# opentrack/neuralnet-tracker-traincode

Hardware: AMD Instinct MI355X
Metric: face-crops/sec fwd+bwd @ batch 512 (higher is better)
Workload: dtype f32; 1 GPU; NetworkWithPointHead(mobilenetv1, point head on, NLL off = training-script defaults): zero_grad + fwd + multi-task loss + bwd + fused clip/Adam step; per_gpu_batch=512, global_batch=512, input=129x129x1 f32, parallelism=dp1

## Files before the change

include/ttk.h:

```cpp
#ifndef TTK_H_
#define TTK_H_

#include <stddef.h>
#include <stdint.h>

#ifdef __cplusplus
extern "C" {
#endif

typedef void* ttk_stream_t;

#define TTK_ABI_VERSION 31

enum {
  TTK_BN_SCALE = 0,
  TTK_BN_BETA = 1,
  TTK_BN_MEAN = 2,
  TTK_BN_RSTD = 3,
  TTK_BN_GA = 4,
  TTK_BN_GB = 5,
  TTK_BN_GMEAN = 6,
  TTK_BN_AUX = 7,
  TTK_BN_ROWS = 8
};
enum { TTK_AUX_ACT_BOUND = 0, TTK_AUX_DY_BOUND = 1, TTK_AUX_GMAX = 2 };
#define TTK_STORE_ACT_BF16 1
#define TTK_STORE_GRAD_BF16 2
#define TTK_LAYOUT_ROWS 4
#define TTK_LAYOUT_CB64 8
#define TTK_MAX_PARTIAL_ROWS_ELEMENTWISE 1024
#define TTK_GEMM_BLOCK_M 128

int ttk_abi_version(void);
const char* ttk_last_error_string(void);
int ttk_clear_error(void);

int ttk_partial_rows_elementwise(int64_t work_items);
int ttk_partial_rows_dwconv(int B, int H, int W, int C, int stride, int backward);
int ttk_partial_rows_gemm(int64_t M);
int ttk_partial_rows_pwconv(int64_t M, int K, int Nout, int dgrad);
int ttk_pwconv_tile_rows(int64_t M, int K, int Nout, int dgrad);

int ttk_bn_fwd_finalize(float* part, const float* pivot, int part_rows, int C, int64_t count,
                        const float* gamma, const float* beta,
                        float* running_mean, float* running_var, int64_t* num_batches_tracked,
                        float momentum, float eps, float* bn, ttk_stream_t stream);
int ttk_bn_eval_prepare(const float* gamma, const float* beta, const float* running_mean,
                        const float* running_var, float eps, int C, float* bn, ttk_stream_t stream);
int ttk_bn_bwd_finalize(float* part, int part_rows, int C, int64_t count, const float* gamma,
                        float* bn, float* dgamma, float* dbeta, int accumulate, ttk_stream_t stream);

int ttk_bn_bwd_frozen(float* bn, int C, ttk_stream_t stream);
int ttk_bn_frozen_bound(float* part, const float* pivot, int part_rows, int C, int64_t count, float* bn, ttk_stream_t stream);

int ttk_stem_fwd(const float* x, const float* w, void* y, float* part, const float* pivot, int B, int H, int W,
                 int act_bf16, ttk_stream_t stream);
size_t ttk_stem_wgrad_partial_bytes(void);
int ttk_stem_bwd_weight(const void* g, const void* y, const float* bn, const float* x, float* dw,
                        int accumulate, float* partial, int B, int H, int W, int act_bf16,
                        ttk_stream_t stream);

int ttk_dwconv3x3_fwd(const float* yprev, const float* bn_prev, const float* skip_prev, float* a_out,
                      const float* w, float* y, float* part, const float* pivot, int B, int H, int W, int C,
                      int stride, int act_bf16, ttk_stream_t stream);
int ttk_dwconv3x3_bwd_data(const float* g_dw, const float* y_dw, const float* bn_dw, const float* w,
                           const float* skip_grad, const float* yprev, float* bn_prev,
                           const float* skip_prev, const float* a_in, float* g_prev, float* part,
                           float* dw, int dw_accumulate, float* dw_partial, int B, int H, int W, int C,
                           int stride, int act_bf16, ttk_stream_t stream);

int ttk_pwconv1x1_fwd(const float* ydw, const float* bn_dw, const float* w, float* y, float* part, const float* pivot,
                      int64_t M, int Cin, int Cout, void* wsplit, int act_bf16, ttk_stream_t stream);
int ttk_pwconv1x1_bwd_data(const float* g, const float* y, const float* bn_pw, const float* wt,
                           const float* ydw, const float* bn_dw, float* g_dw, float* part, int64_t M,
                           int Cin, int Cout, void* wsplit, int act_bf16, ttk_stream_t stream);
size_t ttk_pwconv_wgrad_partial_bytes(int64_t M, int Cin, int Cout);
size_t ttk_pwconv_wgrad_scratch_bytes(int64_t M, int Cin, int Cout);
int ttk_pwconv1x1_bwd_weight(const float* g, const float* y, const float* bn_pw, const float* ydw,
                             const float* bn_dw, float* dw, float* partial, int64_t M, int Cin, int Cout,
                             int act_bf16, ttk_stream_t stream);
int ttk_pwconv1x1_bwd_fused_rows(int64_t M, int Cin, int Cout);
size_t ttk_pwconv1x1_bwd_fused_partial_bytes(int64_t M, int Cin, int Cout);
int ttk_pwconv1x1_bwd_fused(const float* g, const float* y, const float* bn_pw, const float* w, const void* wsplit,
                            const float* ydw, const float* bn_dw, float* g_dw, float* dw, float* partial, float* part,
                            int64_t M, int Cin, int Cout, ttk_stream_t stream);
size_t ttk_pwconv_prepared_bytes(int Cin, int Cout);
int ttk_pwconv_prepare_weights(int n, const float* const* w, const int* cin, const int* cout,
                               void* const* prepared, ttk_stream_t stream);
int ttk_transpose(const float* in, float* out, int rows, int cols, ttk_stream_t stream);

int ttk_avgpool_fwd(const float* y, const float* bn, const float* skip, float* feat, int B, int HW,
                    int C, int act_bf16, ttk_stream_t stream);
int ttk_avgpool_bwd(const float* gfeat, const float* y, float* bn, const float* skip, float* g,
                    float* part, int B, int HW, int C, int act_bf16, ttk_stream_t stream);
int ttk_bn_act(const float* y, const float* bn, const float* skip, float* a, int64_t rows, int C,
               ttk_stream_t stream);

int ttk_anyc_partial_rows(int64_t pixels);
int ttk_anyc_stem_fwd(const float* x, const float* w, float* y, float* part, const float* pivot, int B, int H, int W, int Cout,
                      ttk_stream_t stream);
size_t ttk_anyc_stem_wgrad_scratch_bytes(int B, int H, int W, int Cout);
int ttk_anyc_stem_bwd_weight(const float* g, const float* y, const float* bn, const float* x, float* dw, int accumulate, float* scratch, int B,
                             int H, int W, int Cout, ttk_stream_t stream);
int ttk_anyc_dw_fwd(const float* yprev, const float* bn_prev, const float* skip_prev, float* a_out, const float* w, float* y, float* part,
                    const float* pivot, int B, int H, int W, int C, int stride, ttk_stream_t stream);
size_t ttk_anyc_dw_wgrad_scratch_bytes(int B, int H, int W, int C);
int ttk_anyc_dw_bwd_data(const float* g_dw, const float* y_dw, const float* bn_dw, const float* w, const float* skip_grad, const float* yprev,
                         float* bn_prev, const float* skip_prev, const float* a_in, float* g_prev, float* part, float* dw, int dw_accumulate,
                         float* dw_scratch, int B, int H, int W, int C, int stride, ttk_stream_t stream);
int ttk_anyc_pw_fwd(const float* ydw, const float* bn_dw, const float* w, float* y, float* part, const float* pivot, int64_t M, int Cin, int Cout,
                    ttk_stream_t stream);
int ttk_anyc_pw_bwd_data(const float* g, const float* y, const float* bn_pw, const float* w, const float* ydw, float* bn_dw, float* g_dw,
                         float* part, int64_t M, int Cin, int Cout, ttk_stream_t stream);
size_t ttk_anyc_pw_wgrad_scratch_bytes(int64_t M, int Cin, int Cout);
int ttk_anyc_pw_bwd_weight(const float* g, const float* y, const float* bn_pw, const float* ydw, const float* bn_dw, float* dw, int accumulate,
                           float* scratch, int64_t M, int Cin, int Cout, ttk_stream_t stream);
int ttk_anyc_avgpool_fwd(const float* y, const float* bn, const float* skip, float* feat, int B, int HW, int C, ttk_stream_t stream);
int ttk_anyc_avgpool_bwd(const float* gfeat, const float* y, float* bn, const float* skip, float* g, float* part, int B, int HW, int C,
                         ttk_stream_t stream);
int ttk_anyc_bn_act(const float* y, const float* bn, const float* skip, float* a, int64_t rows, int C, ttk_stream_t stream);

size_t ttk_bc_prepared_bytes(int Cin, int Cout);
int ttk_bc_prepare_weights(int n, const float* const* w, const int* cin, const int* cout, void* const* prepared, ttk_stream_t stream);
int ttk_bc_partial_rows_pw(int64_t M, int K, int Nout);
int ttk_bc_partial_rows_dw(int B, int H, int W, int C, int stride, int backward);
int ttk_bc_pw_fwd(const void* ydw, const float* bn_dw, const void* wprep, void* y, float* part, const float* pivot, int64_t M, int Cin,
                  int Cout, ttk_stream_t stream);
int ttk_bc_pw_bwd_data(const void* g, const void* y, const float* bn_pw, const void* wprep, const void* ydw, const float* bn_dw,
                       void* g_dw, float* part, int64_t M, int Cin, int Cout, ttk_stream_t stream);
size_t ttk_bc_pw_wgrad_scratch_bytes(int64_t M, int Cin, int Cout);
int ttk_bc_pw_bwd_weight(const void* g, const void* y, const float* bn_pw, const void* ydw, const float* bn_dw, float* dw,
                         float* scratch, int64_t M, int Cin, int Cout, ttk_stream_t stream);
int ttk_bc_pw_wgrad_slices(int64_t M, int Cin, int Cout);
int ttk_bc_pw_bwd_fused_rows(int64_t M, int Cin, int Cout);
size_t ttk_bc_pw_bwd_fused_scratch_bytes(int64_t M, int Cin, int Cout);
int ttk_bc_pw_bwd_fused(const void* g, const void* y, const float* bn_pw, const void* wprep, const void* ydw, const float* bn_dw,
                        void* g_dw, float* dw, float* scratch, float* part, int64_t M, int Cin, int Cout, ttk_stream_t stream);
int ttk_bc_partial_rows_pool(int B, int HW, int C);
int ttk_bc_avgpool_fwd(const void* y, const float* bn, const void* skip, float* feat, int B, int HW, int C, ttk_stream_t stream);
int ttk_bc_avgpool_bwd(const float* gfeat, const void* y, const float* bn, const void* skip, void* g, float* part, int B, int HW, int C,
                       ttk_stream_t stream);
int ttk_bc_dw_fwd(const void* yprev, const float* bn_prev, const void* skip_prev, void* a_out, const float* w, void* y, float* part,
                  const float* pivot, int B, int H, int W, int C, int stride, ttk_stream_t stream);
int ttk_bc_dw_bwd_data(const void* g_dw, const void* y_dw, const float* bn_dw, const float* w, const void* skip_grad,
                       const void* yprev, const float* bn_prev, const void* skip_prev, const void* a_in, void* g_prev, float* part,
                       float* dw, int dw_accumulate, float* dw_partial, int B, int H, int W, int C, int stride, ttk_stream_t stream);
int ttk_bc_bn_bwd_finalize_fold(float* part, int part_rows, int C, int64_t count, const float* gamma, float* bn, float* dgamma, float* dbeta,
                                int accumulate, const float* fold_partial, int fold_rows, int64_t fold_n, float* fold_out, int fold_accumulate,
                                ttk_stream_t stream);

int ttk_conv_weight_repack(const float* w, void* w_fwd, void* w_bwd, int Cout, int Cin, int KH, int KW,
                           ttk_stream_t stream);
int ttk_conv_prepare_weights(int n, const float* const* w, void* const* w_fwd, void* const* w_bwd, const int* cout,
                             const int* cin, const int* ksize, ttk_stream_t stream);
int ttk_conv_fwd(const float* a_in, const float* a_bound, const void* w_fwd, float* y, float* part, const float* pivot, int B, int H,
                 int W, int Cin, int Cout, int KH, int KW, int stride, int pad, ttk_stream_t stream);
int ttk_conv_bwd_data(const float* g, const float* y, const float* bn, const void* w_bwd, const float* mask_y,
                      float* mask_bn, float* g_in, float* part, int B, int H, int W, int Cin, int Cout,
                      int KH, int KW, int stride, int pad, ttk_stream_t stream);
size_t ttk_conv_wgrad_partial_bytes(int B, int H, int W, int Cin, int Cout, int KH, int KW, int stride, int pad);
int ttk_conv_bwd_weight(const float* g, const float* y, const float* bn, const float* a_in, const float* a_bound, float* dw,
                        float* partial, int B, int H, int W, int Cin, int Cout, int KH, int KW, int stride, int pad, ttk_stream_t stream);

int ttk_stem7_fwd(const float* x, const float* w, float* y, float* part, const float* pivot, int B, int H, int W, ttk_stream_t stream);
size_t ttk_stem7_wgrad_partial_bytes(int B, int H, int W);
int ttk_stem7_bwd_weight(const float* g, const float* y, const float* bn, const float* x, float* dw, float* partial, int B,
                         int H, int W, ttk_stream_t stream);
int ttk_maxpool3x3s2_fwd(const float* y, float* bn, float* a, unsigned char* idx, int B, int H, int W, int C,
                         ttk_stream_t stream);
int ttk_maxpool3x3s2_bwd(const float* ga, const float* gb, const unsigned char* idx, const float* y, const float* bn,
                         float* g, float* part, int B, int H, int W, int C, ttk_stream_t stream);
int ttk_bn_add_act(const float* y, float* bn, const float* res, const float* res_bn, float* a, const float* res_bound,
                   int measure, int64_t rows, int C, ttk_stream_t stream);
int ttk_bn_bwd_apply(const float* g, const float* y, const float* bn, void* dy, int64_t rows, int C, ttk_stream_t stream);
int ttk_blur3x3_fwd(const float* a, float* t, int B, int H, int W, int C, int stride, ttk_stream_t stream);
int ttk_blur3x3_bwd(const float* ga, const float* gb, float* g, int B, int H, int W, int C, int stride, ttk_stream_t stream);
int ttk_residual_bwd(const float* ga, const float* gb, const float* a, const float* y, float* bn, const float* yd,
                     float* bnd, float* gs, float* part, float* partd, int64_t rows, int C, ttk_stream_t stream);

int ttk_heads_num_rows(int enable_uncertainty, int enable_point_head, int enable_6drot);
int ttk_heads_fwd(const float* feat, const float* wcat, const float* bcat, const int* ids,
                  const float* P, const float* Pk, const float* keypts, const float* keyeig, int B, int F,
                  int NZ, int enable_uncertainty, int enable_point_head, int use_offset, int enable_6drot,
                  float* z, float* roi, float* coord, float* rot, float* qu, float* Lc, float* Lr, float* pts,
                  float* shp, ttk_stream_t stream);
int ttk_heads_bwd(const float* feat, const float* wcat, const float* z, const int* ids, const float* P,
                  const float* Pk, const float* keypts, const float* keyeig, int B, int F, int NZ,
                  int enable_uncertainty, int enable_point_head, int use_offset, int enable_6drot,
                  const float* g_roi, const float* g_coord, const float* g_rot, const float* g_qu,
                  const float* g_Lc, const float* g_Lr, const float* g_pts, const float* g_shp, float* dz,
                  float* dprow, float* dfeat, float* dwcat, float* dbcat, float* dP, float* dPk,
                  ttk_stream_t stream);
int ttk_diag_scale_fwd(const float* hidden, float* out, int n, ttk_stream_t stream);
int ttk_diag_scale_bwd(const float* hidden, const float* gout, float* ghidden, int n, ttk_stream_t stream);

int ttk_loss_rot_fwd(const float* q, const float* t, int n, float* v, ttk_stream_t stream);
int ttk_loss_rot_bwd(const float* q, const float* t, const float* gv, int n, float* gq, ttk_stream_t stream);
int ttk_loss_rot6d_fwd(const float* R, const float* t, int n, float* v, ttk_stream_t stream);
int ttk_loss_rot6d_bwd(const float* t, const float* gv, int n, float* gR, ttk_stream_t stream);
int ttk_loss_ortho6d_fwd(const float* z6, int n, float* v, ttk_stream_t stream);
int ttk_loss_ortho6d_bwd(const float* z6, const float* gv, int n, float* gz6, ttk_stream_t stream);
int ttk_mat_to_quat_fwd(const float* m, int n, float* q, ttk_stream_t stream);
int ttk_mat_to_quat_bwd(const float* m, const float* gq, int n, float* gm, ttk_stream_t stream);
int ttk_loss_quatreg_fwd(const float* q, int n, float* v, ttk_stream_t stream);
int ttk_loss_quatreg_bwd(const float* q, const float* gv, int n, float* gq, ttk_stream_t stream);
int ttk_loss_mse_rows_fwd(const float* p, const float* t, int n, int D, float* v, ttk_stream_t stream);
int ttk_loss_mse_rows_bwd(const float* p, const float* t, const float* gv, int n, int D, float* gp, ttk_stream_t stream);
int ttk_loss_mse_cols_fwd(const float* p, const float* t, int n, int Dt, int c0, int Dc, float* v, ttk_stream_t stream);
int ttk_loss_mse_cols_bwd(const float* p, const float* t, const float* gv, int n, int Dt, int c0, int Dc, float* gp, ttk_stream_t stream);
int ttk_multi_copy(int n, const float* const* src, float* const* dst, const int64_t* count, ttk_stream_t stream);
int ttk_weighted_sum_fwd(int n, const float* const* val, const float* const* sample_w, const float* w, const int* count,
                         float scale, float* out, ttk_stream_t stream);
int ttk_weighted_sum_bwd(int n, const float* gout, const float* const* sample_w, const float* w, const int* count,
                         float scale, float* const* gval, ttk_stream_t stream);
int ttk_loss_points_fwd(const float* p, const float* t, int n, int dim, float chin, float eye, float* v, ttk_stream_t stream);
int ttk_loss_points_bwd(const float* p, const float* t, const float* gv, int n, int dim, float chin, float eye, float* gp, ttk_stream_t stream);
int ttk_loss_nllrot_fwd(const float* q, const float* t, const float* L, int n, float* v, ttk_stream_t stream);
int ttk_loss_nllrot_bwd(const float* q, const float* t, const float* L, const float* gv, int n, float* gq, float* gL, ttk_stream_t stream);
int ttk_loss_nllcoord_fwd(const float* c, const float* t, const float* L, int n, float* v, ttk_stream_t stream);
int ttk_loss_nllcoord_bwd(const float* c, const float* t, const float* L, const float* gv, int n, float* gc, float* gL, ttk_stream_t stream);
int ttk_loss_normal_fwd(const float* mu, const float* sigma, const float* x, int n, int per, int points, int dim, float chin, float eye, float* v, ttk_stream_t stream);
int ttk_loss_normal_bwd(const float* mu, const float* sigma, const float* x, const float* gv, int n, int per, int points, int dim, float chin, float eye, float* gmu, float* gsigma, ttk_stream_t stream);
enum { TTK_ELEM_L2 = 0, TTK_ELEM_L1 = 1, TTK_ELEM_SMOOTH_L1 = 2 };
int ttk_loss_laplace_fwd(const float* mu, const float* b, const float* x, int n, int per, int points, int dim, float chin, float eye, float* v, ttk_stream_t stream);
int ttk_loss_laplace_bwd(const float* mu, const float* b, const float* x, const float* gv, int n, int per, int points, int dim, float chin, float eye, float* gmu, float* gb, ttk_stream_t stream);
int ttk_loss_elem_fwd(const float* p, const float* t, const float* colw, int n, int D, int kind, float beta, float* v, ttk_stream_t stream);
int ttk_loss_elem_bwd(const float* p, const float* t, const float* colw, const float* gv, int n, int D, int kind, float beta, float* gp, ttk_stream_t stream);
int ttk_loss_rot_geodesic_fwd(const float* q, const float* t, int n, float* v, ttk_stream_t stream);
int ttk_loss_rot_geodesic_bwd(const float* q, const float* t, const float* gv, int n, float* gq, ttk_stream_t stream);
int ttk_loss_gmm_fwd(const float* x, const double* ck, const double* mu, const double* sinv, int K, double fudge, int n, float* v, double* post, ttk_stream_t stream);
int ttk_loss_gmm_bwd(const float* x, const double* mu, const double* sinv, const double* post, int K, double fudge, const float* gv, int n, float* gx, ttk_stream_t stream);

#define TTK_LOSS_BATCH_MAX 32
enum {
  TTK_OP_ROT_FWD, TTK_OP_ROT_BWD, TTK_OP_ROT6D_FWD, TTK_OP_ROT6D_BWD, TTK_OP_ORTHO6D_FWD, TTK_OP_ORTHO6D_BWD,
  TTK_OP_QUATREG_FWD, TTK_OP_QUATREG_BWD, TTK_OP_MSE_ROWS_FWD, TTK_OP_MSE_ROWS_BWD, TTK_OP_MSE_COLS_FWD, TTK_OP_MSE_COLS_BWD,
  TTK_OP_POINTS_FWD, TTK_OP_POINTS_BWD, TTK_OP_NLLROT_FWD, TTK_OP_NLLROT_BWD, TTK_OP_NLLCOORD_FWD, TTK_OP_NLLCOORD_BWD,
  TTK_OP_NORMAL_FWD, TTK_OP_NORMAL_BWD, TTK_OP_GMM_FWD, TTK_OP_GMM_BWD, TTK_OP_COUNT
};
typedef struct ttk_loss_op {
  int kind;
  int items;
  const void* p[6];
  int i[4];
  float f[2];
  double d;
} ttk_loss_op;
int ttk_loss_batch(int nops, const ttk_loss_op* ops, ttk_stream_t stream);

int ttk_loss_batch_rows(int nops, const ttk_loss_op* ops, const unsigned* tag_sets, const int* tag_code, ttk_stream_t stream);
int ttk_row_weights(const float* wtable, const int* tag_code, const float* dataset_weight, int K, int n, float* rw, ttk_stream_t stream);

#define TTK_INTENSITY_EQUALIZE 0
#define TTK_INTENSITY_POSTERIZE_BITS 1
#define TTK_INTENSITY_GAMMA 2
#define TTK_INTENSITY_CONTRAST 3
#define TTK_INTENSITY_BRIGHTNESS 4
#define TTK_INTENSITY_BLUR 5
#define TTK_INTENSITY_NOISE_STD 6
#define TTK_INTENSITY_PARAMS 8
int ttk_intensity_augment(const float* x, float* y, const float* params, const float* noise, int B, int H, int W,
                          float out_shift, ttk_stream_t stream);

#define TTK_ADAM_MAX_GROUPS 128
#define TTK_ADAM_HYPER_LR 0
#define TTK_ADAM_HYPER_WD 128
#define TTK_ADAM_HYPER_FLOATS 256
int ttk_clip_adam(const int64_t* ptrs, const int32_t* numel, const int32_t* group,
                  const int32_t* chunk_tensor, const int32_t* chunk_offset, int nchunks, int chunk_size,
                  const float* lr4, const float* wd4, float beta1, float beta2, float eps, float max_norm,
                  float grad_scale, float* steps, float* partial, float* out_norm, const float* hyper_dev,
                  ttk_stream_t stream);

int ttk_view_roi(const float* face_roi, const float* scales, const float* translations,
                 float beyond_border_shift, int B, int* view_roi, ttk_stream_t stream);
int ttk_roi_transform(const int* view_roi, const float* angles, int B, int N, float* tr, ttk_stream_t stream);
int ttk_affine_warp(const void* src, int src_is_u8, int B, int Hs, int Ws, const float* tr, float* out,
                    int N, float mul, float add, ttk_stream_t stream);
int ttk_area_crop(const void* src, int src_is_u8, int B, int Hs, int Ws, const float* tr, float* out,
                  int N, float mul, float add, ttk_stream_t stream);
int ttk_affine_labels(const float* tr, int B, int N, float* coord, float* pose, float* roi,
                      const float* pts_in, float* pts_out, ttk_stream_t stream);

int ttk_stream_probe(const float* src, float* dst, float* sink, int64_t rows, int row_bytes, int seg_bytes, int nread, int nwrite,
                     int64_t stream_bytes, int unroll, int nontemporal, int blocks, ttk_stream_t stream);

#ifdef __cplusplus
}
#endif
#endif
```

neuralnet-tracker-traincode_amd/csrc/dwconv_tiled.hip:

```cpp
#include "ttk_common.h"
#include <type_traits>
#ifndef TTK_DW_FWD_U
#define TTK_DW_FWD_U 6
#endif
#ifndef TTK_DW_BWD_U
#define TTK_DW_BWD_U 4
#endif
#ifndef TTK_DW_FWD_U2
#define TTK_DW_FWD_U2 6
#endif

namespace ttk {

#ifndef TTK_DW_LDS_PIX
#define TTK_DW_LDS_PIX 368
#endif
constexpr int kLdsPixBudget32 = TTK_DW_LDS_PIX;
__host__ __device__ constexpr int lds_pix_budget(int SL) { return kLdsPixBudget32 * 32 / SL; }
__host__ __device__ constexpr int ilog2(int v) { return v <= 1 ? 0 : 1 + ilog2(v >> 1); }
#ifndef TTK_DW_WGS_PER_CU
#define TTK_DW_WGS_PER_CU 3
#endif
constexpr int kMaxDwBlocks = 256 * TTK_DW_WGS_PER_CU;
constexpr int kFwdUSkip = 4, kFwdUPlain = TTK_DW_FWD_U, kFwdUPlain2 = TTK_DW_FWD_U2;

struct DwTiling {
  int SL;
  int R, nbands, nslabs, grid, rows;
  int NI;
  int stage_rows;
  int NCT, TW;
  int carry;
};
#ifndef TTK_DW_CARRY
#define TTK_DW_CARRY 1
#endif
#ifndef TTK_DW_CARRY_BWD
#define TTK_DW_CARRY_BWD 1
#endif
constexpr int kCarryRegs = 5;

constexpr int kColTileMinW = 48;
constexpr int kColTile = 17;

__host__ __device__ inline int dw_band_rows(int Hgrid, int Wstage, int stride, bool backward, int SL = 32) {
  const int stage_rows = lds_pix_budget(SL) / (Wstage + 2);
  int R;
  if (!backward) R = (stage_rows - 3) / stride + 1;
  else R = (stride == 1) ? stage_rows - 2 : 2 * (stage_rows - 2);
  if (R < 1) R = 1;
  if (R > Hgrid) R = Hgrid;
  return R;
}

inline DwTiling dw_tiling_sl(int B, int H, int W, int C, int stride, bool backward, int SL) {
  const int Ho = (H - 1) / stride + 1, Wo = (W - 1) / stride + 1;
  DwTiling t;
  t.SL = SL;
  t.NCT = 1;
  t.TW = Wo;
  static const int col_tile = [] { const char* e = exp_env("TTK_DW_COLTILE"); return e ? atoi(e) : kColTile; }();
  static const int carry_bwd = [] { const char* e = exp_env("TTK_DW_CARRY_BWD"); return e ? atoi(e) : TTK_DW_CARRY_BWD; }();
  t.carry = backward ? (carry_bwd && stride == 1 && (Wo + 2) <= 80)
                     : (TTK_DW_CARRY && (3 - stride) * (W + 2) * (SL / 4) <= kCarryRegs * kBlock);
  if (!t.carry && stride == 1 && W >= kColTileMinW && col_tile < W) {
    t.NCT = (W + col_tile - 1) / col_tile;
    t.TW = (W + t.NCT - 1) / t.NCT;
  }
  const int Wtile = t.NCT > 1 ? t.TW : (backward ? Wo : W);
  t.R = backward ? dw_band_rows(H, Wtile, stride, true, SL) : dw_band_rows(Ho, Wtile, stride, false, SL);
  t.nbands = ((backward ? H : Ho) + t.R - 1) / t.R;
  t.nslabs = C / SL;
  t.stage_rows = backward ? (stride == 1 ? t.R + 2 : t.R / 2 + 2) : (t.R - 1) * stride + 3;
  t.NI = 1;
  if (t.nbands == 1) t.carry = 0;
  if (t.nbands == 1 && t.NCT == 1) {
    const int per_image = t.stage_rows * ((backward ? Wo : W) + 2);
    t.NI = lds_pix_budget(SL) / per_image;
    if (t.NI > B) t.NI = B;
    if (t.NI < 1) t.NI = 1;
  }
  int64_t tiles_per_slab = (int64_t)((B + t.NI - 1) / t.NI) * t.nbands * t.NCT;
  int64_t rows = kMaxDwBlocks / t.nslabs;
  if (rows < 1) rows = 1;
  if (rows > tiles_per_slab) rows = tiles_per_slab;
  t.rows = (int)rows;
  t.grid = t.rows * t.nslabs;
  return t;
}

inline DwTiling dw_tiling(int B, int H, int W, int C, int stride, bool backward) {
  return dw_tiling_sl(B, H, W, C, stride, backward, kCB);
}

struct TileDiv {
  float inv;
  unsigned d;
  __device__ __forceinline__ explicit TileDiv(unsigned d_) : inv(1.0f / (float)d_), d(d_) {}
  __device__ __forceinline__ unsigned div(unsigned n) const { return (unsigned)(((float)n + 0.5f) * inv); }
};

struct SlabWeights {
  float v[36];
  __device__ __forceinline__ void load(const float* w, int c) {
    const float4* p = reinterpret_cast<const float4*>(w + 9 * c);
#pragma unroll
    for (int i = 0; i < 9; ++i) {
      const float4 q = p[i];
      v[4 * i] = q.x; v[4 * i + 1] = q.y; v[4 * i + 2] = q.z; v[4 * i + 3] = q.w;
    }
  }
  __device__ __forceinline__ float4 tap(int t) const { return make_float4(v[t], v[9 + t], v[18 + t], v[27 + t]); }
};

template <int SL>
__device__ __forceinline__ float4 slab_wave_fold(float4 v) {
#pragma unroll
  for (int off = SL / 4; off < kWave; off <<= 1) {
    v.x += __shfl_xor(v.x, off); v.y += __shfl_xor(v.y, off);
    v.z += __shfl_xor(v.z, off); v.w += __shfl_xor(v.w, off);
  }
  return v;
}

struct D4 {
  double x, y, z, w;
  __device__ __forceinline__ void add(float4 v) { x += v.x; y += v.y; z += v.z; w += v.w; }
  __device__ __forceinline__ void addmul(float4 a, float4 b) {
    x += (double)a.x * b.x; y += (double)a.y * b.y; z += (double)a.z * b.z; w += (double)a.w * b.w;
  }
};
__device__ __forceinline__ double shfl_xor_d(double v, int off) {
  int lo = __double2loint(v), hi = __double2hiint(v);
  lo = __shfl_xor(lo, off);
  hi = __shfl_xor(hi, off);
  return __hiloint2double(hi, lo);
}
template <int SL>
__device__ __forceinline__ D4 slab_wave_fold_d(D4 v) {
#pragma unroll
  for (int off = SL / 4; off < kWave; off <<= 1) {
    v.x += shfl_xor_d(v.x, off); v.y += shfl_xor_d(v.y, off);
    v.z += shfl_xor_d(v.z, off); v.w += shfl_xor_d(v.w, off);
  }
  return v;
}

template <int SL>
__device__ __forceinline__ void slab_partials(D4 s1, D4 s2, int q, int C, int c_slab, float* part_row, float* red_f) {
  double* red = reinterpret_cast<double*>(red_f);
  s1 = slab_wave_fold_d<SL>(s1);
  s2 = slab_wave_fold_d<SL>(s2);
  const int lane = threadIdx.x & 63, wv = threadIdx.x >> 6;
  __syncthreads();
  if (lane < SL / 4) {
    double* d = red + (wv * 2 + 0) * SL + 4 * q;
    d[0] = s1.x; d[1] = s1.y; d[2] = s1.z; d[3] = s1.w;
    d = red + (wv * 2 + 1) * SL + 4 * q;
    d[0] = s2.x; d[1] = s2.y; d[2] = s2.z; d[3] = s2.w;
  }
  __syncthreads();
  if (threadIdx.x < 2 * SL) {
    const int which = threadIdx.x / SL, c = threadIdx.x % SL;
    double a = 0.0;
    for (int w = 0; w < kBlock / kWave; ++w) a += red[(w * 2 + which) * SL + c];
    part_row[(size_t)which * C + c_slab + c] = (float)a;
  }
}

template <int S, bool SKIP, int SL, bool CARRY>
__global__ void __launch_bounds__(kBlock) __attribute__((amdgpu_waves_per_eu(TTK_DW_WGS_PER_CU, TTK_DW_WGS_PER_CU)))
dw_fwd_tiled_k(const float* __restrict__ yprev, const float* __restrict__ bn_prev,
                                                          const float* __restrict__ skip_prev, float* __restrict__ a_out,
                                                          const float* __restrict__ w, float* __restrict__ y,
                                                          float* __restrict__ part, const float* __restrict__ pivot, int B, int H, int W, int C,
                                                          int Ho, int Wo, int R, int nbands, int nslabs, int NI_, int NCT_, int TW) {
  extern __shared__ __attribute__((aligned(16))) float lds[];
  constexpr int kSlab = SL, kSlabQuads = SL / 4, kPixSlots = kBlock / kSlabQuads, kQs = ilog2(kSlabQuads), kPs = ilog2(SL);
  const int tid = threadIdx.x, q = tid & (kSlabQuads - 1), slot = tid >> kQs;
  const int slab = blockIdx.x % nslabs, c0 = slab * kSlab + 4 * q;
  static_assert(SL == kCB, "a slab is one channel block of the activation layout");
  constexpr int cshift = 5;
  SlabWeights wr;
  wr.load(w, c0);
  const BnApply4 bn = BnApply4::load(bn_prev, C, c0);
  const float4 pv = pivot ? ld4(pivot + c0) : f4(0.f);
  D4 s1{0.0, 0.0, 0.0, 0.0}, s2{0.0, 0.0, 0.0, 0.0};
  const int NI = CARRY ? 1 : NI_, NCT = CARRY ? 1 : NCT_;
  constexpr bool carry = CARRY;
  const unsigned tiles = (unsigned)((B + NI - 1) / NI) * nbands * NCT;
  const unsigned wgs = gridDim.x / nslabs, wg = blockIdx.x / nslabs;
  const unsigned t_begin = carry ? (unsigned)((uint64_t)tiles * wg / wgs) : wg, t_end = carry ? (unsigned)((uint64_t)tiles * (wg + 1) / wgs) : tiles;
  const unsigned t_step = carry ? 1u : wgs;
  int prev_img = -1, prev_band = -2, prev_nrows = 0;
  constexpr int OV = 3 - S;
  for (unsigned t = t_begin; t < t_end; t += t_step) {
    const unsigned tb = t / (unsigned)NCT, ti = tb / (unsigned)nbands;
    const int ct = (int)(t - tb * NCT), band = (int)(tb - ti * nbands), n0 = (int)ti * NI;
    const int nimg = min(NI, B - n0);
    const int cx0 = ct * TW, tw = NCT > 1 ? min(TW, Wo - cx0) : Wo;
    const int Wp = NCT > 1 ? tw + 2 : W + 2;
    const int o0 = band * R, o1 = min(o0 + R, Ho);
    const int i0 = o0 * S - 1;
    const int nrows = (o1 - 1 - o0) * S + 3;
    const unsigned PI = (unsigned)(nrows * Wp);
    const TileDiv dPI(PI), dWp((unsigned)Wp), dtw((unsigned)tw);
    const size_t tin = ((size_t)slab * B * H * W + (size_t)n0 * H * W) * kCB, tout = ((size_t)slab * B * Ho * Wo + (size_t)n0 * Ho * Wo) * kCB;
    const float* ytile = yprev + tin;
    const float* sktile = SKIP ? skip_prev + tin : nullptr;
    float* aotile = a_out ? a_out + tin : nullptr;
    float* youttile = y + tout;
    const int ov = (carry && (int)ti == prev_img && band == prev_band + 1) ? OV : 0;
    const int own_hi = (carry && t + 1 < t_end && band + 1 < nbands) ? i0 + nrows : o1;
    float4 cr[kCarryRegs];
    const int ncopy = ov * Wp * kSlabQuads;
    if (ov) {
      const float* src = lds + (size_t)(prev_nrows - OV) * Wp * kSlab;
#pragma unroll
      for (int u = 0; u < kCarryRegs; ++u)
        if (tid + u * kBlock < ncopy) cr[u] = ld4(src + (size_t)(tid + u * kBlock) * 4);
    }
    prev_img = (int)ti; prev_band = band; prev_nrows = nrows;
    __syncthreads();
    if (ov) {
#pragma unroll
      for (int u = 0; u < kCarryRegs; ++u)
        if (tid + u * kBlock < ncopy) st4(lds + (size_t)(tid + u * kBlock) * 4, cr[u]);
    }
    const int nstage = nimg * ((int)PI - ov * Wp) * kSlabQuads;
    const unsigned ovpix = (unsigned)(ov * Wp);
    constexpr int kFwdU = SKIP ? kFwdUSkip : (S == 2 ? kFwdUPlain2 : (CARRY ? kFwdUPlain - 1 : kFwdUPlain));
    for (int e = tid; e < nstage; e += kFwdU * kBlock) {
      float4 yv[kFwdU], sk[SKIP ? kFwdU : 1];
      unsigned off[kFwdU];
      bool in[kFwdU];
      int pxs[kFwdU], rows[kFwdU];
#pragma unroll
      for (int u = 0; u < kFwdU; ++u) {
        const int ee = e + u * kBlock;
        const unsigned pxa = ((unsigned)ee >> kQs) + ovpix;
        const unsigned img = NI > 1 ? dPI.div(pxa) : 0u, px = NI > 1 ? pxa - __umul24(img, PI) : pxa;
        const unsigned prow = dWp.div(px);
        const int col = (int)(px - __umul24(prow, (unsigned)Wp)) - 1 + cx0, row = i0 + (int)prow;
        pxs[u] = (int)pxa;
        rows[u] = (row >= o0 && row < own_hi && col >= cx0 && col < cx0 + tw) ? 1 : 0;
        in[u] = ee < nstage && row >= 0 && row < H && col >= 0 && col < W;
        off[u] = in[u] ? ((__umul24(__umul24(img, (unsigned)H) + (unsigned)row, (unsigned)W) + (unsigned)col) << cshift) + 4 * q : 0u;
        yv[u] = in[u] ? ld4nt(ytile + off[u]) : f4(0.f);
        if constexpr (SKIP) sk[u] = in[u] ? ld4nt(sktile + off[u]) : f4(0.f);
      }
#pragma unroll
      for (int u = 0; u < kFwdU; ++u) {
        const int ee = e + u * kBlock;
        if (ee >= nstage) break;
        float4 a = f4(0.f);
        if (in[u]) {
          if constexpr (SKIP) a = bn.act(yv[u], sk[u]);
          else a = bn.act(yv[u]);
          if (S == 1 && a_out && rows[u]) st4(aotile + off[u], a);
        }
        st4(lds + (size_t)pxs[u] * kSlab + 4 * q, a);
      }
    }
    __syncthreads();
    const unsigned npix1 = (unsigned)((o1 - o0) * tw);
    const int npix = nimg * (int)npix1;
    const TileDiv dnp(npix1);
    for (int p = slot; p < npix; p += kPixSlots) {
      const unsigned img = NI > 1 ? dnp.div((unsigned)p) : 0u, pp = NI > 1 ? (unsigned)p - __umul24(img, npix1) : (unsigned)p;
      const unsigned prow = dtw.div(pp);
      const int ho = o0 + (int)prow, wl = (int)(pp - __umul24(prow, (unsigned)tw)), wo = cx0 + wl;
      const float* base = lds + ((__umul24(img, PI) + __umul24(prow * S, (unsigned)Wp) + (unsigned)(wl * S)) << kPs) + 4 * q;
      float4 acc = f4(0.f);
#pragma unroll
      for (int kh = 0; kh < 3; ++kh)
#pragma unroll
        for (int kw = 0; kw < 3; ++kw) acc = fma4(ld4(base + ((size_t)kh * Wp + kw) * kSlab), wr.tap(kh * 3 + kw), acc);
      st4(youttile + ((__umul24(__umul24(img, (unsigned)Ho) + (unsigned)ho, (unsigned)Wo) + (unsigned)wo) << cshift) + 4 * q, acc);
      acc = sub4(acc, pv);
      s1.add(acc);
      s2.addmul(acc, acc);
    }
  }
  if (part) {
    const int stage = NI * ((R - 1) * S + 3) * (NCT > 1 ? TW + 2 : W + 2) * kSlab;
    slab_partials<SL>(s1, s2, q, C, slab * kSlab, part + (size_t)(blockIdx.x / nslabs) * 2 * C, lds + stage);
  }
}

#ifndef TTK_DW_BWD_LEAN_PIX
#define TTK_DW_BWD_LEAN_PIX 4
#endif
#ifndef TTK_DW_BWD_LEAN_PIX2
#define TTK_DW_BWD_LEAN_PIX2 4
#endif
template <int S, int SL, bool LEAN, bool CARRY>
__global__ void __launch_bounds__(kBlock) __attribute__((amdgpu_waves_per_eu(TTK_DW_WGS_PER_CU, TTK_DW_WGS_PER_CU)))
dw_bwd_tiled_k(const float* __restrict__ g_dw, const float* __restrict__ y_dw,
                                                          const float* __restrict__ bn_dw, const float* __restrict__ w,
                                                          const float* __restrict__ skip_grad,
                                                          const float* __restrict__ yprev, float* __restrict__ bn_prev,
                                                          const float* __restrict__ skip_prev, const float* __restrict__ a_in,
                                                          float* __restrict__ g_prev, float* __restrict__ part,
                                                          float* __restrict__ dwgrad, float* __restrict__ dw_partial, int B, int H, int W, int C, int Ho, int Wo,
                                                          int R, int nbands, int nslabs, int stage_floats, int NI_, int NCT_, int TW, int ring) {
  extern __shared__ __attribute__((aligned(16))) float lds[];
  const int NI = CARRY ? 1 : NI_, NCT = CARRY ? 1 : NCT_;
  constexpr int kSlab = SL, kSlabQuads = SL / 4, kPixSlots = kBlock / kSlabQuads, kQs = ilog2(kSlabQuads), kPs = ilog2(SL);
  const int tid = threadIdx.x, q = tid & (kSlabQuads - 1), slot = tid >> kQs;
  const int slab = blockIdx.x % nslabs, c0 = slab * kSlab + 4 * q;
  float* wt = lds + stage_floats + 4 * 9 * kSlab;
  if (slot == 0) {
#pragma unroll
    for (int t = 0; t < 9; ++t)
      st4(wt + t * kSlab + 4 * q, make_float4(w[(size_t)(c0 + 0) * 9 + t], w[(size_t)(c0 + 1) * 9 + t], w[(size_t)(c0 + 2) * 9 + t], w[(size_t)(c0 + 3) * 9 + t]));
  }
  static_assert(SL == kCB, "a slab is one channel block of the activation layout");
  constexpr int cshift = 5;
  const BnApply4 bnp = BnApply4::load(bn_prev, C, c0);
  const BnGrad4 bg = BnGrad4::load(bn_dw, C, c0);
  D4 s1{0.0, 0.0, 0.0, 0.0}, s2{0.0, 0.0, 0.0, 0.0};
  float gmx = 0.f;
  float4 wacc[9];
#pragma unroll
  for (int t = 0; t < 9; ++t) wacc[t] = f4(0.f);
  const unsigned tiles = (unsigned)((B + NI - 1) / NI) * nbands * NCT;
  const unsigned wgs = gridDim.x / nslabs, wg = blockIdx.x / nslabs;
  const unsigned t_begin = CARRY ? (unsigned)((uint64_t)tiles * wg / wgs) : wg, t_end = CARRY ? (unsigned)((uint64_t)tiles * (wg + 1) / wgs) : tiles;
  const unsigned t_step = CARRY ? 1u : wgs;
  int prev_img = -1, prev_band = -2, prev_hi = -1;
  for (unsigned t = t_begin; t < t_end; t += t_step) {
    const unsigned tb = t / (unsigned)NCT, ti = tb / (unsigned)nbands;
    const int ct = (int)(t - tb * NCT), band = (int)(tb - ti * nbands), n0 = (int)ti * NI;
    const int nimg = min(NI, B - n0);
    const int cx0 = ct * TW, tw = NCT > 1 ? min(TW, W - cx0) : W;
    const int Wp = NCT > 1 ? tw + 2 : Wo + 2;
    const int r0 = band * R, r1 = min(r0 + R, H);
    const int ho_lo = max(0, (r0 - 1 + S - 1) / S * (r0 > 0 ? 1 : 0));
    const int ho_hi = min(Ho - 1, r1 / S);
    const int nrows = ho_hi - ho_lo + 1;
    const unsigned PI = (unsigned)(nrows * Wp);
    const TileDiv dPI(PI), dWp((unsigned)Wp), dtw((unsigned)tw);
    const size_t tdy = ((size_t)slab * B * Ho * Wo + (size_t)n0 * Ho * Wo) * kCB, tin = ((size_t)slab * B * H * W + (size_t)n0 * H * W) * kCB;
    const float* gtile = g_dw + tdy;
    const float* ydtile = y_dw + tdy;
    const float* yptile = yprev + tin;
    const float* aitile = a_in ? a_in + tin : nullptr;
    const float* sktile = skip_prev ? skip_prev + tin : nullptr;
    const float* sgtile = skip_grad ? skip_grad + tin : nullptr;
    float* gptile = g_prev + tin;
    const int ov = (CARRY && (int)ti == prev_img && band == prev_band + 1 && prev_hi >= ho_lo) ? prev_hi - ho_lo + 1 : 0;
    const int rbase = CARRY ? ho_lo % ring : 0;
    prev_img = (int)ti; prev_band = band; prev_hi = ho_hi;
    __syncthreads();
    const unsigned ovpix = (unsigned)(ov * Wp);
    const int nstage = nimg * ((int)PI - (int)ovpix) * kSlabQuads;
    constexpr int kBwdU = TTK_DW_BWD_U;
    for (int e = tid; e < nstage; e += kBwdU * kBlock) {
      float4 gv[kBwdU], yv[kBwdU];
      bool in[kBwdU];
      unsigned pxs[kBwdU];
#pragma unroll
      for (int u = 0; u < kBwdU; ++u) {
        const int ee = e + u * kBlock;
        const unsigned pxa = ((unsigned)ee >> kQs) + ovpix;
        const unsigned img = NI > 1 ? dPI.div(pxa) : 0u, px = NI > 1 ? pxa - __umul24(img, PI) : pxa;
        const unsigned prow = dWp.div(px);
        const int col = (int)(px - __umul24(prow, (unsigned)Wp)) - 1 + cx0, row = ho_lo + (int)prow;
        if constexpr (CARRY) {
          unsigned rr = (unsigned)rbase + prow;
          rr -= rr >= (unsigned)ring ? (unsigned)ring : 0u;
          pxs[u] = __umul24(rr, (unsigned)Wp) + (px - __umul24(prow, (unsigned)Wp));
        } else {
          pxs[u] = pxa;
        }
        in[u] = ee < nstage && col >= 0 && col < Wo;
        const unsigned off = in[u] ? ((__umul24(__umul24(img, (unsigned)Ho) + (unsigned)row, (unsigned)Wo) + (unsigned)col) << cshift) + 4 * q : 0u;
        gv[u] = in[u] ? ld4nt(gtile + off) : f4(0.f);
        yv[u] = in[u] ? ld4nt(ydtile + off) : f4(0.f);
      }
#pragma unroll
      for (int u = 0; u < kBwdU; ++u) {
        const int ee = e + u * kBlock;
        if (ee >= nstage) break;
        st4(lds + (size_t)pxs[u] * kSlab + 4 * q, in[u] ? bg.dy(gv[u], yv[u]) : f4(0.f));
      }
    }
    __syncthreads();
    const unsigned npix1 = (unsigned)((r1 - r0) * tw);
    const int npix = nimg * (int)npix1;
    const TileDiv dnp(npix1);
    constexpr int NP = LEAN ? (S == 2 ? TTK_DW_BWD_LEAN_PIX2 : TTK_DW_BWD_LEAN_PIX) : 2;
    for (int p = slot; p < npix; p += NP * kPixSlots) {
      bool has[NP];
      unsigned imgs[NP], offs[NP];
      int his[NP], wis[NP];
      float4 yps[NP], raws[NP], sgs[NP];
#pragma unroll
      for (int j = 0; j < NP; ++j) {
        const int pj = p + j * kPixSlots;
        has[j] = pj < npix;
        const unsigned pq = has[j] ? (unsigned)pj : (unsigned)p;
        imgs[j] = NI > 1 ? dnp.div(pq) : 0u;
        const unsigned pp = NI > 1 ? pq - __umul24(imgs[j], npix1) : pq;
        const unsigned pr = dtw.div(pp);
        his[j] = r0 + (int)pr;
        wis[j] = cx0 + (int)(pp - __umul24(pr, (unsigned)tw));
        offs[j] = ((__umul24(__umul24(imgs[j], (unsigned)H) + (unsigned)his[j], (unsigned)W) + (unsigned)wis[j]) << cshift) + 4 * q;
      }
#pragma unroll
      for (int j = 0; j < NP; ++j) yps[j] = ld4nt(yptile + offs[j]);
#pragma unroll
      for (int j = 0; j < NP; ++j) {
        raws[j] = f4(0.f);
        sgs[j] = f4(0.f);
        if (!LEAN) {
          if (a_in) raws[j] = ld4nt(aitile + offs[j]);
          else if (skip_prev) raws[j] = ld4nt(sktile + offs[j]);
          if (skip_grad) sgs[j] = ld4nt(sgtile + offs[j]);
        }
      }
#pragma unroll
      for (int j = 0; j < NP; ++j) {
        if (j > 0 && !has[j]) break;
        const int hi = his[j], wi = wis[j];
        const float* dyimg = lds + (__umul24(imgs[j], PI) << kPs);
        const float4 yp = yps[j], raw = raws[j], sg = sgs[j];
        float4 a;
        if (!LEAN && a_in) a = raw;
        else a = (!LEAN && skip_prev) ? bnp.act(yp, raw) : bnp.act(yp);
        float4 G = f4(0.f);
#pragma unroll
        for (int kh = 0; kh < 3; ++kh) {
          const int th = hi + 1 - kh;
          if (th < 0 || (S == 2 && (th & 1))) continue;
          const int ho = th / S;
          if (ho > Ho - 1) continue;
#pragma unroll
          for (int kw = 0; kw < 3; ++kw) {
            const int tw = wi + 1 - kw;
            if (S == 2 && (tw & 1)) continue;
            const int wo = (S == 1) ? tw : (tw >> 1);
            int lr = ho - ho_lo;
            if constexpr (CARRY) { lr += rbase; lr -= lr >= ring ? ring : 0; }
            const float4 dy = ld4(dyimg + ((__mul24(lr, Wp) + wo - cx0 + 1) << kPs) + 4 * q);
            G = fma4(dy, ld4(wt + (kh * 3 + kw) * kSlab + 4 * q), G);
            wacc[kh * 3 + kw] = fma4(dy, a, wacc[kh * 3 + kw]);
          }
        }
        if (!LEAN && skip_grad) G = add4(G, sg);
        const float4 gp = mask4(G, a);
        st4(gptile + offs[j], gp);
        gmx = fmaxf(fmaxf(gmx, fmaxf(fabsf(gp.x), fabsf(gp.y))), fmaxf(fabsf(gp.z), fabsf(gp.w)));
        s1.add(gp);
        s2.addmul(gp, sub4(yp, bnp.mean));
      }
    }
  }
  float* red = lds + stage_floats;
#pragma unroll
  for (int off = 32; off >= 1; off >>= 1) gmx = fmaxf(gmx, __shfl_xor(gmx, off));
  if ((tid & 63) == 0) {
    unsigned* slot = reinterpret_cast<unsigned*>(bn_prev + (size_t)TTK_BN_AUX * C + TTK_AUX_GMAX);
    if (__float_as_uint(gmx) > __hip_atomic_load(slot, __ATOMIC_RELAXED, __HIP_MEMORY_SCOPE_AGENT)) atomicMax(slot, __float_as_uint(gmx));
  }
  if (part) slab_partials<SL>(s1, s2, q, C, slab * kSlab, part + (size_t)(blockIdx.x / nslabs) * 2 * C, red);
  if (dwgrad) {
    __syncthreads();
    const int lane = tid & 63, wv = tid >> 6;
#pragma unroll
    for (int t = 0; t < 9; ++t) {
      const float4 v = slab_wave_fold<SL>(wacc[t]);
      if (lane < kSlabQuads) st4(red + ((size_t)wv * 9 + t) * kSlab + 4 * q, v);
    }
    __syncthreads();
    for (int i = tid; i < 9 * kSlab; i += kBlock) {
      const int t = i / kSlab, c = i % kSlab;
      float a = 0.f;
      for (int wq = 0; wq < kBlock / kWave; ++wq) a += red[((size_t)wq * 9 + t) * kSlab + c];
      if (dw_partial) dw_partial[((size_t)(blockIdx.x / nslabs) * C + slab * kSlab + c) * 9 + t] = a;
      else atomicAdd(dwgrad + (size_t)(slab * kSlab + c) * 9 + t, a);
    }
  }
}

__global__ void zero_fill_k(float* p, int64_t n) {
  const int64_t i = (int64_t)blockIdx.x * blockDim.x + threadIdx.x;
  if (i < n) p[i] = 0.f;
}

template <typename F>
static void with_flag(bool b, F&& f) {
  if (b) f(std::true_type{});
  else f(std::false_type{});
}

static bool dw_shape_ok2(int B, int H, int W, int C, int stride) {
  return B > 0 && H > 0 && W > 0 && W <= 256 && C >= 32 && C <= 1024 && (C & (C - 1)) == 0 && (stride == 1 || stride == 2);
}

}

using namespace ttk;

extern "C" {

int ttk_partial_rows_dwconv(int B, int H, int W, int C, int stride, int backward) {
  if (!dw_shape_ok2(B, H, W, C, stride)) return -1;
  return dw_tiling(B, H, W, C, stride, backward != 0).rows;
}

int ttk_dwconv3x3_fwd(const float* yprev, const float* bn_prev, const float* skip_prev, float* a_out, const float* w, float* y,
                      float* part, const float* pivot, int B, int H, int W, int C, int stride, int act_bf16, ttk_stream_t stream) {
  TTK_REQUIRE(yprev && bn_prev && w && y, "dwconv3x3_fwd: null pointer");
  TTK_REQUIRE(dw_shape_ok2(B, H, W, C, stride), "dwconv3x3_fwd: unsupported shape B=%d H=%d W=%d C=%d stride=%d (C: power of two in 32..1024, W <= 256)", B, H, W, C, stride);
  TTK_REQUIRE(!(a_out && stride != 1), "dwconv3x3_fwd: a_out requires stride 1");
  TTK_REQUIRE_FP32_STORAGE(act_bf16, "dwconv3x3_fwd");
  const int Ho = (H - 1) / stride + 1, Wo = (W - 1) / stride + 1;
  const DwTiling t = dw_tiling(B, H, W, C, stride, false);
  TTK_REQUIRE((int64_t)((B + t.NI - 1) / t.NI) * t.nbands * t.NCT < ((int64_t)1 << 31), "dwconv3x3_fwd: too many tiles for 32-bit indexing");
  const size_t stage = (size_t)t.NI * t.stage_rows * ((t.NCT > 1 ? t.TW : W) + 2) * t.SL;
  const size_t sm = (stage + 16 * t.SL) * sizeof(float);
  with_flag(stride == 2, [&](auto s2) {
    with_flag(skip_prev != nullptr, [&](auto skip) {
      with_flag(t.carry != 0, [&](auto carry) {
        hipLaunchKernelGGL((dw_fwd_tiled_k<decltype(s2)::value ? 2 : 1, decltype(skip)::value, kCB, decltype(carry)::value>), dim3(t.grid), dim3(kBlock), sm,
                           (hipStream_t)stream, yprev, bn_prev, skip_prev, a_out, w, y, part, pivot, B, H, W, C, Ho, Wo, t.R, t.nbands, t.nslabs, t.NI,
                           t.NCT, t.TW);
      });
    });
  });
  TTK_LAUNCH_CHECK("dwconv3x3_fwd");
}

int ttk_dwconv3x3_bwd_data(const float* g_dw, const float* y_dw, const float* bn_dw, const float* w, const float* skip_grad,
                           const float* yprev, float* bn_prev, const float* skip_prev, const float* a_in, float* g_prev,
                           float* part, float* dw, int dw_accumulate, float* dw_partial, int B, int H, int W, int C, int stride,
                           int act_bf16, ttk_stream_t stream) {
  TTK_REQUIRE(g_dw && y_dw && bn_dw && w && yprev && bn_prev && g_prev, "dwconv3x3_bwd_data: null pointer");
  TTK_REQUIRE(dw_shape_ok2(B, H, W, C, stride), "dwconv3x3_bwd_data: unsupported shape");
  TTK_REQUIRE(!(skip_grad && stride != 1), "dwconv3x3_bwd_data: residual gradient requires stride 1");
  TTK_REQUIRE_FP32_STORAGE(act_bf16, "dwconv3x3_bwd_data");
  const int Ho = (H - 1) / stride + 1, Wo = (W - 1) / stride + 1;
  const DwTiling t = dw_tiling(B, H, W, C, stride, true);
  TTK_REQUIRE((int64_t)((B + t.NI - 1) / t.NI) * t.nbands * t.NCT < ((int64_t)1 << 31), "dwconv3x3_bwd_data: too many tiles for 32-bit indexing");
  const size_t stage = (size_t)t.NI * t.stage_rows * ((t.NCT > 1 ? t.TW : Wo) + 2) * t.SL;
  const size_t sm = (stage + 4 * 9 * t.SL + 9 * t.SL) * sizeof(float);
  hipStream_t st = (hipStream_t)stream;
  if (!dw) dw_partial = nullptr;
  TTK_REQUIRE(dw_accumulate != 2 || dw_partial, "dwconv3x3_bwd_data: dw_accumulate = 2 (rows folded by the caller) needs dw and dw_partial");
  if (dw && !dw_accumulate && !dw_partial) hipLaunchKernelGGL(zero_fill_k, dim3((9 * C + 255) / 256), dim3(256), 0, st, dw, (int64_t)9 * C);
  with_flag(stride == 2, [&](auto s2) {
    with_flag(!a_in && !skip_prev && !skip_grad, [&](auto lean) {
      with_flag(t.carry != 0, [&](auto carry) {
        hipLaunchKernelGGL((dw_bwd_tiled_k<decltype(s2)::value ? 2 : 1, kCB, decltype(lean)::value, decltype(carry)::value>), dim3(t.grid), dim3(kBlock), sm, st,
                           g_dw, y_dw, bn_dw, w, skip_grad, yprev, bn_prev, skip_prev, a_in, g_prev, part, dw, dw_partial, B, H, W, C, Ho, Wo, t.R,
                           t.nbands, t.nslabs, (int)stage, t.NI, t.NCT, t.TW, t.stage_rows);
      });
    });
  });
  if (dw_partial && dw_accumulate != 2) launch_fold_partials(dw_partial, t.rows, (int64_t)9 * C, dw, dw_accumulate, st);
  TTK_LAUNCH_CHECK("dwconv3x3_bwd_data");
}

}
```

neuralnet-tracker-traincode_amd/csrc/pool.hip:

```cpp
#include "ttk_common.h"

namespace ttk {

__device__ __forceinline__ size_t pool_off(int layout, int64_t m, int c, int64_t M, int C) {
  if (layout == 1) return (size_t)m * C + c;
  if (layout == 2) return ((size_t)(c >> 6) * (size_t)M + (size_t)m) * 64 + (c & 63);
  return act_off(m, c, M);
}

__global__ void __launch_bounds__(kBlock) avgpool_fwd_k(const float* __restrict__ y, const float* __restrict__ bnp,
                                                         const float* __restrict__ skip,
                                                         float* __restrict__ feat, int B, int HW, int C, int rows_layout) {
  const int quads = C >> 2;
  const int64_t items = (int64_t)B * quads;
  const float inv = 1.0f / (float)HW;
  for (int64_t idx = (int64_t)blockIdx.x * kBlock + threadIdx.x; idx < items; idx += (int64_t)gridDim.x * kBlock) {
    const int c4 = (int)(idx % quads);
    const int n = (int)(idx / quads);
    const BnApply4 bn = BnApply4::load(bnp, C, 4 * c4);
    float4 s = f4(0.f);
    for (int p = 0; p < HW; ++p) {
      const int64_t m = (int64_t)n * HW + p;
      const size_t off = pool_off(rows_layout, m, 4 * c4, (int64_t)B * HW, C);
      s = add4(s, skip ? bn.act(ld4(y + off), ld4(skip + off)) : bn.act(ld4(y + off)));
    }
    st4(feat + (size_t)n * C + 4 * c4, make_float4(s.x * inv, s.y * inv, s.z * inv, s.w * inv));
  }
}

__global__ void __launch_bounds__(kBlock) avgpool_bwd_k(const float* __restrict__ gfeat, const float* __restrict__ y,
                                                         float* __restrict__ bnp, const float* __restrict__ skip, float* __restrict__ g,
                                                         float* __restrict__ part, int B, int HW, int C, int qshift, int rows_layout) {
  extern __shared__ __attribute__((aligned(16))) float smem[];
  const int quads = C >> 2;
  const int c4 = threadIdx.x & (quads - 1);
  const BnApply4 bn = BnApply4::load(bnp, C, 4 * c4);
  const float inv = 1.0f / (float)HW;
  const int64_t items = ((int64_t)B * HW) << qshift;
  float4 s1 = f4(0.f), s2 = f4(0.f);
  float gmx = 0.f;
  for (int64_t idx = (int64_t)blockIdx.x * kBlock + threadIdx.x; idx < items; idx += (int64_t)gridDim.x * kBlock) {
    const int n = (int)((unsigned)(idx >> qshift) / (unsigned)HW);
    const size_t off = pool_off(rows_layout, idx >> qshift, 4 * c4, (int64_t)B * HW, C);
    const float4 yv = ld4(y + off);
    const float4 a = skip ? bn.act(yv, ld4(skip + off)) : bn.act(yv);
    float4 gv = ld4(gfeat + (size_t)n * C + 4 * c4);
    gv = mask4(make_float4(gv.x * inv, gv.y * inv, gv.z * inv, gv.w * inv), a);
    st4(g + off, gv);
    gmx = fmaxf(fmaxf(gmx, fmaxf(fabsf(gv.x), fabsf(gv.y))), fmaxf(fabsf(gv.z), fabsf(gv.w)));
    s1 = add4(s1, gv);
    s2 = fma4(gv, sub4(yv, bn.mean), s2);
  }
#pragma unroll
  for (int off = 32; off >= 1; off >>= 1) gmx = fmaxf(gmx, __shfl_xor(gmx, off));
  if ((threadIdx.x & 63) == 0) {
    unsigned* slot = reinterpret_cast<unsigned*>(bnp + (size_t)TTK_BN_AUX * C + TTK_AUX_GMAX);
    if (__float_as_uint(gmx) > __hip_atomic_load(slot, __ATOMIC_RELAXED, __HIP_MEMORY_SCOPE_AGENT)) atomicMax(slot, __float_as_uint(gmx));
  }
  if (part) block_channel_partials<1024>(s1, s2, c4, C, part + (size_t)blockIdx.x * 2 * C, smem);
}

}

using namespace ttk;

static int pool_layout(int flags) { return (flags & TTK_LAYOUT_ROWS) ? 1 : ((flags & TTK_LAYOUT_CB64) ? 2 : 0); }

static int log2i_(int v) {
  int r = 0;
  while ((1 << r) < v) ++r;
  return r;
}

extern "C" {

int ttk_avgpool_fwd(const float* y, const float* bn, const float* skip, float* feat, int B, int HW,
                    int C, int act_bf16, ttk_stream_t stream) {
  TTK_REQUIRE(y && bn && feat, "avgpool_fwd: null pointer");
  TTK_REQUIRE(B > 0 && HW > 0 && C >= 32 && C <= 1024 && (C & (C - 1)) == 0, "avgpool_fwd: unsupported shape B=%d HW=%d C=%d", B, HW, C);
  TTK_REQUIRE_FP32_STORAGE(act_bf16, "avgpool_fwd");
  const int64_t items = (int64_t)B * (C / 4);
  hipLaunchKernelGGL(avgpool_fwd_k, dim3(elementwise_grid(items)), dim3(kBlock), 0, (hipStream_t)stream, y, bn, skip, feat, B, HW, C,
                     pool_layout(act_bf16));
  TTK_LAUNCH_CHECK("avgpool_fwd");
}

int ttk_avgpool_bwd(const float* gfeat, const float* y, float* bn, const float* skip, float* g,
                    float* part, int B, int HW, int C, int act_bf16, ttk_stream_t stream) {
  TTK_REQUIRE(gfeat && y && bn && g, "avgpool_bwd: null pointer");
  TTK_REQUIRE(B > 0 && HW > 0 && C >= 32 && C <= 1024 && (C & (C - 1)) == 0, "avgpool_bwd: unsupported shape");
  TTK_REQUIRE((int64_t)B * HW < (int64_t)1 << 31, "avgpool_bwd: too many pixels for 32-bit indexing");
  TTK_REQUIRE_FP32_STORAGE(act_bf16, "avgpool_bwd");
  const int qs = log2i_(C / 4);
  const int64_t items = ((int64_t)B * HW) << qs;
  hipLaunchKernelGGL(avgpool_bwd_k, dim3(elementwise_grid(items)), dim3(kBlock), 2 * (size_t)C * sizeof(float), (hipStream_t)stream, gfeat, y, bn,
                     skip, g, part, B, HW, C, qs, pool_layout(act_bf16));
  TTK_LAUNCH_CHECK("avgpool_bwd");
}

}
```

neuralnet-tracker-traincode_amd/trackertraincode/_hip.py:

```python
from __future__ import annotations

import functools

import ctypes
import os
from ctypes import c_char_p, c_double, c_float, c_int, c_int64, c_void_p

import torch

_HERE = os.path.dirname(os.path.abspath(__file__))
LIB_PATH = os.environ.get("TTK_LIB") or os.path.join(os.path.dirname(_HERE), "libttk_hip.so")

_P, _I, _L, _F, _D = c_void_p, c_int, c_int64, c_float, c_double

_SIGNATURES = {
    "ttk_bn_fwd_finalize": [_P, _P, _I, _I, _L, _P, _P, _P, _P, _P, _F, _F, _P],
    "ttk_bn_bwd_frozen": [_P, _I],
    "ttk_bn_frozen_bound": [_P, _P, _I, _I, _L, _P],
    "ttk_bn_eval_prepare": [_P, _P, _P, _P, _F, _I, _P],
    "ttk_bn_bwd_finalize": [_P, _I, _I, _L, _P, _P, _P, _P, _I],
    "ttk_stem_fwd": [_P, _P, _P, _P, _P, _I, _I, _I, _I],
    "ttk_stem_bwd_weight": [_P, _P, _P, _P, _P, _I, _P, _I, _I, _I, _I],
    "ttk_dwconv3x3_fwd": [_P] * 8 + [_I] * 6,
    "ttk_dwconv3x3_bwd_data": [_P] * 12 + [_I, _P] + [_I] * 6,
    "ttk_pwconv1x1_fwd": [_P, _P, _P, _P, _P, _P, _L, _I, _I, _P, _I],
    "ttk_pwconv1x1_bwd_data": [_P] * 8 + [_L, _I, _I, _P, _I],
    "ttk_pwconv1x1_bwd_weight": [_P] * 7 + [_L, _I, _I, _I],
    "ttk_pwconv_prepare_weights": [_I, _P, _P, _P, _P],
    "ttk_pwconv1x1_bwd_fused": [_P] * 11 + [_L, _I, _I],
    "ttk_transpose": [_P, _P, _I, _I],
    "ttk_avgpool_fwd": [_P, _P, _P, _P, _I, _I, _I, _I],
    "ttk_avgpool_bwd": [_P, _P, _P, _P, _P, _P, _I, _I, _I, _I],
    "ttk_bn_act": [_P, _P, _P, _P, _L, _I],
    "ttk_stem7_fwd": [_P, _P, _P, _P, _P, _I, _I, _I],
    "ttk_stem7_bwd_weight": [_P, _P, _P, _P, _P, _P, _I, _I, _I],
    "ttk_maxpool3x3s2_fwd": [_P, _P, _P, _P, _I, _I, _I, _I],
    "ttk_maxpool3x3s2_bwd": [_P] * 7 + [_I] * 4,
    "ttk_bn_add_act": [_P, _P, _P, _P, _P, _P, _I, _L, _I],
    "ttk_residual_bwd": [_P] * 10 + [_L, _I],
    "ttk_bn_bwd_apply": [_P, _P, _P, _P, _L, _I],
    "ttk_conv_weight_repack": [_P, _P, _P, _I, _I, _I, _I],
    "ttk_conv_prepare_weights": [_I, _P, _P, _P, _P, _P, _P],
    "ttk_conv_fwd": [_P, _P, _P, _P, _P, _P] + [_I] * 9,
    "ttk_conv_bwd_data": [_P] * 8 + [_I] * 9,
    "ttk_conv_bwd_weight": [_P] * 7 + [_I] * 9,
    "ttk_heads_fwd": [_P] * 8 + [_I] * 7 + [_P] * 9,
    "ttk_heads_bwd": [_P] * 8 + [_I] * 7 + [_P] * 15,
    "ttk_diag_scale_fwd": [_P, _P, _I],
    "ttk_diag_scale_bwd": [_P, _P, _P, _I],
    "ttk_loss_rot_fwd": [_P, _P, _I, _P],
    "ttk_loss_rot_bwd": [_P, _P, _P, _I, _P],
    "ttk_loss_rot6d_fwd": [_P, _P, _I, _P],
    "ttk_loss_rot6d_bwd": [_P, _P, _I, _P],
    "ttk_loss_ortho6d_fwd": [_P, _I, _P],
    "ttk_loss_ortho6d_bwd": [_P, _P, _I, _P],
    "ttk_mat_to_quat_fwd": [_P, _I, _P],
    "ttk_mat_to_quat_bwd": [_P, _P, _I, _P],
    "ttk_loss_quatreg_fwd": [_P, _I, _P],
    "ttk_loss_quatreg_bwd": [_P, _P, _I, _P],
    "ttk_loss_mse_rows_fwd": [_P, _P, _I, _I, _P],
    "ttk_loss_mse_rows_bwd": [_P, _P, _P, _I, _I, _P],
    "ttk_loss_mse_cols_fwd": [_P, _P, _I, _I, _I, _I, _P],
    "ttk_loss_mse_cols_bwd": [_P, _P, _P, _I, _I, _I, _I, _P],
    "ttk_multi_copy": [_I, _P, _P, _P],
    "ttk_weighted_sum_fwd": [_I, _P, _P, _P, _P, _F, _P],
    "ttk_weighted_sum_bwd": [_I, _P, _P, _P, _P, _F, _P],
    "ttk_loss_points_fwd": [_P, _P, _I, _I, _F, _F, _P],
    "ttk_loss_points_bwd": [_P, _P, _P, _I, _I, _F, _F, _P],
    "ttk_loss_nllrot_fwd": [_P, _P, _P, _I, _P],
    "ttk_loss_nllrot_bwd": [_P, _P, _P, _P, _I, _P, _P],
    "ttk_loss_nllcoord_fwd": [_P, _P, _P, _I, _P],
    "ttk_loss_nllcoord_bwd": [_P, _P, _P, _P, _I, _P, _P],
    "ttk_loss_normal_fwd": [_P, _P, _P, _I, _I, _I, _I, _F, _F, _P],
    "ttk_loss_normal_bwd": [_P, _P, _P, _P, _I, _I, _I, _I, _F, _F, _P, _P],
    "ttk_loss_laplace_fwd": [_P, _P, _P, _I, _I, _I, _I, _F, _F, _P],
    "ttk_loss_laplace_bwd": [_P, _P, _P, _P, _I, _I, _I, _I, _F, _F, _P, _P],
    "ttk_loss_elem_fwd": [_P, _P, _P, _I, _I, _I, _F, _P],
    "ttk_loss_elem_bwd": [_P, _P, _P, _P, _I, _I, _I, _F, _P],
    "ttk_loss_rot_geodesic_fwd": [_P, _P, _I, _P],
    "ttk_loss_rot_geodesic_bwd": [_P, _P, _P, _I, _P],
    "ttk_loss_gmm_fwd": [_P, _P, _P, _P, _I, _D, _I, _P, _P],
    "ttk_loss_gmm_bwd": [_P, _P, _P, _P, _I, _D, _P, _I, _P],
    "ttk_loss_batch": [_I, _P],
    "ttk_loss_batch_rows": [_I, _P, _P, _P],
    "ttk_row_weights": [_P, _P, _P, _I, _I, _P],
    "ttk_blur3x3_fwd": [_P, _P, _I, _I, _I, _I, _I],
    "ttk_blur3x3_bwd": [_P, _P, _P, _I, _I, _I, _I, _I],
    "ttk_view_roi": [_P, _P, _P, _F, _I, _P],
    "ttk_roi_transform": [_P, _P, _I, _I, _P],
    "ttk_affine_warp": [_P, _I, _I, _I, _I, _P, _P, _I, _F, _F],
    "ttk_area_crop": [_P, _I, _I, _I, _I, _P, _P, _I, _F, _F],
    "ttk_affine_labels": [_P, _I, _I, _P, _P, _P, _P, _P],
    "ttk_intensity_augment": [_P, _P, _P, _P, _I, _I, _I, _F],
    "ttk_clip_adam": [_P, _P, _P, _P, _P, _I, _I, _P, _P, _F, _F, _F, _F, _F, _P, _P, _P, _P],
    "ttk_stream_probe": [_P, _P, _P, _L, _I, _I, _I, _I, _L, _I, _I, _I],
    "ttk_bc_prepare_weights": [_I, _P, _P, _P, _P],
    "ttk_bc_pw_fwd": [_P, _P, _P, _P, _P, _P, _L, _I, _I],
    "ttk_bc_pw_bwd_data": [_P] * 8 + [_L, _I, _I],
    "ttk_bc_pw_bwd_weight": [_P] * 7 + [_L, _I, _I],
    "ttk_bc_pw_bwd_fused": [_P] * 10 + [_L, _I, _I],
    "ttk_bc_dw_fwd": [_P] * 8 + [_I] * 5,
    "ttk_bc_avgpool_fwd": [_P, _P, _P, _P, _I, _I, _I],
    "ttk_bc_avgpool_bwd": [_P, _P, _P, _P, _P, _P, _I, _I, _I],
    "ttk_bc_dw_bwd_data": [_P] * 12 + [_I, _P] + [_I] * 5,
    "ttk_bc_bn_bwd_finalize_fold": [_P, _I, _I, _L, _P, _P, _P, _P, _I, _P, _I, _L, _P, _I],
    "ttk_anyc_stem_fwd": [_P, _P, _P, _P, _P, _I, _I, _I, _I],
    "ttk_anyc_stem_bwd_weight": [_P, _P, _P, _P, _P, _I, _P, _I, _I, _I, _I],
    "ttk_anyc_dw_fwd": [_P] * 8 + [_I] * 5,
    "ttk_anyc_dw_bwd_data": [_P] * 12 + [_I, _P] + [_I] * 5,
    "ttk_anyc_pw_fwd": [_P, _P, _P, _P, _P, _P, _L, _I, _I],
    "ttk_anyc_pw_bwd_data": [_P] * 8 + [_L, _I, _I],
    "ttk_anyc_pw_bwd_weight": [_P] * 6 + [_I, _P, _L, _I, _I],
    "ttk_anyc_avgpool_fwd": [_P, _P, _P, _P, _I, _I, _I],
    "ttk_anyc_avgpool_bwd": [_P, _P, _P, _P, _P, _P, _I, _I, _I],
    "ttk_anyc_bn_act": [_P, _P, _P, _P, _L, _I],
}

ABI_VERSION = 31


BN_PIVOT = True


def bn_pivot() -> bool:
    return BN_PIVOT


class LossOp(ctypes.Structure):
    _fields_ = [("kind", c_int), ("items", c_int), ("p", c_void_p * 6), ("i", c_int * 4), ("f", c_float * 2), ("d", c_double)]


LOSS_BATCH_MAX = 32
_n = lambda k: (lambda a: a[k])
LOSS_BATCH_OPS = {
    "ttk_loss_rot_fwd": (0, _n(2)), "ttk_loss_rot_bwd": (1, _n(3)), "ttk_loss_rot6d_fwd": (2, _n(2)), "ttk_loss_rot6d_bwd": (3, _n(2)),
    "ttk_loss_ortho6d_fwd": (4, _n(1)), "ttk_loss_ortho6d_bwd": (5, _n(2)), "ttk_loss_quatreg_fwd": (6, _n(1)), "ttk_loss_quatreg_bwd": (7, _n(2)),
    "ttk_loss_mse_rows_fwd": (8, lambda a: a[2] * 64), "ttk_loss_mse_rows_bwd": (9, lambda a: a[3] * a[4]),
    "ttk_loss_mse_cols_fwd": (10, lambda a: a[2] * 64), "ttk_loss_mse_cols_bwd": (11, lambda a: a[3] * a[4]),
    "ttk_loss_points_fwd": (12, lambda a: a[2] * 64), "ttk_loss_points_bwd": (13, lambda a: a[3] * 204),
    "ttk_loss_nllrot_fwd": (14, _n(3)), "ttk_loss_nllrot_bwd": (15, _n(4)), "ttk_loss_nllcoord_fwd": (16, _n(3)), "ttk_loss_nllcoord_bwd": (17, _n(4)),
    "ttk_loss_normal_fwd": (18, lambda a: a[3] * 64), "ttk_loss_normal_bwd": (19, lambda a: a[4] * (204 if a[6] else a[5])),
    "ttk_loss_gmm_fwd": (20, lambda a: a[6] * 64), "ttk_loss_gmm_bwd": (21, lambda a: a[7] * 50),
}


class _Library:
    def __init__(self):
        if not os.path.exists(LIB_PATH):
            raise RuntimeError(
                f"{LIB_PATH} not found: the HIP kernels are not built. Run "
                "`python -c 'import __graft_entry__ as g; g.build()'` (or `make -C "
                "neuralnet-tracker-traincode_amd/csrc`). There is no CPU/PyTorch fallback for the training path."
            )
        self.cdll = ctypes.CDLL(LIB_PATH)
        self.cdll.ttk_last_error_string.restype = c_char_p
        self.cdll.ttk_abi_version.restype = c_int
        self.cdll.ttk_clear_error.restype = c_int
        self._clear = self.cdll.ttk_clear_error
        v = self.cdll.ttk_abi_version()
        if v != ABI_VERSION:
            raise RuntimeError(f"libttk_hip.so ABI version {v}, host expects {ABI_VERSION}: rebuild")
        for name in ("ttk_partial_rows_elementwise", "ttk_partial_rows_gemm"):
            fn = getattr(self.cdll, name)
            fn.argtypes, fn.restype = [c_int64], c_int
        self.cdll.ttk_partial_rows_pwconv.argtypes, self.cdll.ttk_partial_rows_pwconv.restype = [c_int64, c_int, c_int, c_int], c_int
        self.cdll.ttk_pwconv_tile_rows.argtypes, self.cdll.ttk_pwconv_tile_rows.restype = [c_int64, c_int, c_int, c_int], c_int
        self.cdll.ttk_heads_num_rows.argtypes, self.cdll.ttk_heads_num_rows.restype = [c_int, c_int, c_int], c_int
        self.cdll.ttk_pwconv_prepared_bytes.argtypes, self.cdll.ttk_pwconv_prepared_bytes.restype = [c_int, c_int], ctypes.c_size_t
        self.cdll.ttk_partial_rows_dwconv.argtypes, self.cdll.ttk_partial_rows_dwconv.restype = [c_int] * 6, c_int
        self.cdll.ttk_pwconv_wgrad_partial_bytes.argtypes, self.cdll.ttk_pwconv_wgrad_partial_bytes.restype = [c_int64, c_int, c_int], ctypes.c_size_t
        self.cdll.ttk_pwconv_wgrad_scratch_bytes.argtypes, self.cdll.ttk_pwconv_wgrad_scratch_bytes.restype = [c_int64, c_int, c_int], ctypes.c_size_t
        self.cdll.ttk_conv_wgrad_partial_bytes.argtypes, self.cdll.ttk_conv_wgrad_partial_bytes.restype = [c_int] * 9, ctypes.c_size_t
        self.cdll.ttk_pwconv1x1_bwd_fused_rows.argtypes, self.cdll.ttk_pwconv1x1_bwd_fused_rows.restype = [c_int64, c_int, c_int], c_int
        self.cdll.ttk_pwconv1x1_bwd_fused_partial_bytes.argtypes, self.cdll.ttk_pwconv1x1_bwd_fused_partial_bytes.restype = [c_int64, c_int, c_int], ctypes.c_size_t
        self.cdll.ttk_stem7_wgrad_partial_bytes.argtypes, self.cdll.ttk_stem7_wgrad_partial_bytes.restype = [c_int] * 3, ctypes.c_size_t
        self.cdll.ttk_stem_wgrad_partial_bytes.argtypes, self.cdll.ttk_stem_wgrad_partial_bytes.restype = [], ctypes.c_size_t
        self.cdll.ttk_bc_prepared_bytes.argtypes, self.cdll.ttk_bc_prepared_bytes.restype = [c_int, c_int], ctypes.c_size_t
        self.cdll.ttk_bc_partial_rows_pw.argtypes, self.cdll.ttk_bc_partial_rows_pw.restype = [c_int64, c_int, c_int], c_int
        self.cdll.ttk_bc_partial_rows_dw.argtypes, self.cdll.ttk_bc_partial_rows_dw.restype = [c_int] * 6, c_int
        self.cdll.ttk_bc_partial_rows_pool.argtypes, self.cdll.ttk_bc_partial_rows_pool.restype = [c_int] * 3, c_int
        self.cdll.ttk_bc_pw_wgrad_scratch_bytes.argtypes, self.cdll.ttk_bc_pw_wgrad_scratch_bytes.restype = [c_int64, c_int, c_int], ctypes.c_size_t
        self.cdll.ttk_bc_pw_bwd_fused_rows.argtypes, self.cdll.ttk_bc_pw_bwd_fused_rows.restype = [c_int64, c_int, c_int], c_int
        self.cdll.ttk_bc_pw_wgrad_slices.argtypes, self.cdll.ttk_bc_pw_wgrad_slices.restype = [c_int64, c_int, c_int], c_int
        self.cdll.ttk_bc_pw_bwd_fused_scratch_bytes.argtypes, self.cdll.ttk_bc_pw_bwd_fused_scratch_bytes.restype = [c_int64, c_int, c_int], ctypes.c_size_t
        self.cdll.ttk_anyc_partial_rows.argtypes, self.cdll.ttk_anyc_partial_rows.restype = [c_int64], c_int
        self.cdll.ttk_anyc_stem_wgrad_scratch_bytes.argtypes, self.cdll.ttk_anyc_stem_wgrad_scratch_bytes.restype = [c_int] * 4, ctypes.c_size_t
        self.cdll.ttk_anyc_dw_wgrad_scratch_bytes.argtypes, self.cdll.ttk_anyc_dw_wgrad_scratch_bytes.restype = [c_int] * 4, ctypes.c_size_t
        self.cdll.ttk_anyc_pw_wgrad_scratch_bytes.argtypes, self.cdll.ttk_anyc_pw_wgrad_scratch_bytes.restype = [c_int64, c_int, c_int], ctypes.c_size_t
        self._fns = {}
        self._stale_reported = False
        for name, sig in _SIGNATURES.items():
            fn = getattr(self.cdll, name)
            fn.argtypes = list(sig) + [c_void_p]
            fn.restype = c_int
            self._fns[name] = fn

    def clear_stale_error(self, where: str = "") -> int:
        stale = self._clear()
        if stale and not self._stale_reported:
            self._stale_reported = True
            import warnings
            warnings.warn(f"a HIP error (hipError_t {stale}) from an earlier launch was pending{' at ' + where if where else ''}; it was dropped, "
                          "not raised", RuntimeWarning, stacklevel=2)
        return stale

    def call(self, name: str, *args):
        rc = self._fns[name](*args, _raw_stream(_cur_device()))
        if rc != 0:
            msg = self.cdll.ttk_last_error_string().decode(errors="replace")
            hint = "" if rc < 0 else " (a positive code is a hipError_t read from the sticky hipGetLastError(): an earlier launch of this step may have left it)"
            raise RuntimeError(f"{name} failed (code {rc}): {msg}{hint}")

    @staticmethod
    def pack_loss_ops(chunk):
        arr = (LossOp * len(chunk))()
        for o, (name, args) in zip(arr, chunk):
            kind, items = LOSS_BATCH_OPS[name]
            o.kind, o.items = kind, int(items(args))
            np_ = ni = nf = 0
            for ty, v in zip(_SIGNATURES[name], args):
                if ty is _P:
                    o.p[np_] = v
                    np_ += 1
                elif ty is _I:
                    o.i[ni] = int(v)
                    ni += 1
                elif ty is _F:
                    o.f[nf] = float(v)
                    nf += 1
                else:
                    o.d = float(v)
        return arr

    def loss_batch(self, ops, tag_sets=None, tag_code=None):
        if tag_code is not None and (tag_code.dtype != torch.int32 or tag_sets is None or len(tag_sets) != len(ops)):
            raise RuntimeError("loss_batch: tag_code must be an int32 tensor and tag_sets must hold one set per op")
        for lo in range(0, len(ops), LOSS_BATCH_MAX):
            chunk = ops[lo:lo + LOSS_BATCH_MAX]
            arr = self.pack_loss_ops(chunk)
            if tag_code is None:
                self.call("ttk_loss_batch", len(chunk), arr)
            else:
                sets = (ctypes.c_uint * len(chunk))(*[int(m) & 0xFFFFFFFF for m in tag_sets[lo:lo + LOSS_BATCH_MAX]])
                self.call("ttk_loss_batch_rows", len(chunk), arr, sets, ptr(tag_code))

    def pwconv_prepared_bytes(self, cin: int, cout: int) -> int:
        return self.cdll.ttk_pwconv_prepared_bytes(cin, cout)

    def conv_wgrad_partial_bytes(self, B, H, W, cin, cout, k, stride) -> int:
        return self.cdll.ttk_conv_wgrad_partial_bytes(B, H, W, cin, cout, k, k, stride, k // 2)

    def pwconv_wgrad_partial_bytes(self, m: int, cin: int, cout: int) -> int:
        return self.cdll.ttk_pwconv_wgrad_partial_bytes(m, cin, cout)

    @functools.lru_cache(maxsize=None)
    def pwconv_wgrad_scratch_bytes(self, m: int, cin: int, cout: int) -> int:
        return self.cdll.ttk_pwconv_wgrad_scratch_bytes(m, cin, cout)

    def conv_prepare_weights(self, weights, w_fwd, w_bwd):
        n = len(weights)
        PA, IA = c_void_p * n, c_int * n
        self.call("ttk_conv_prepare_weights", n, PA(*[ptr(w) for w in weights]), PA(*[ptr(t) for t in w_fwd]), PA(*[ptr(t) for t in w_bwd]),
                  IA(*[int(w.shape[0]) for w in weights]), IA(*[int(w.shape[1]) for w in weights]), IA(*[int(w.shape[2]) for w in weights]))

    def pwconv_prepare_weights(self, weights, prepared):
        n = len(weights)
        wp = (c_void_p * n)(*[ptr(w) for w in weights])
        pp = (c_void_p * n)(*[ptr(q) for q in prepared])
        ci = (c_int * n)(*[int(w.shape[1]) for w in weights])
        co = (c_int * n)(*[int(w.shape[0]) for w in weights])
        self.call("ttk_pwconv_prepare_weights", n, wp, ci, co, pp)

    def bc_prepare_weights(self, weights, prepared):
        n = len(weights)
        wp = (c_void_p * n)(*[ptr(w) for w in weights])
        pp = (c_void_p * n)(*[ptr(q) for q in prepared])
        ci = (c_int * n)(*[int(w.shape[1]) for w in weights])
        co = (c_int * n)(*[int(w.shape[0]) for w in weights])
        self.call("ttk_bc_prepare_weights", n, wp, ci, co, pp)

    def multi_copy(self, srcs, dsts):
        for i in range(0, len(dsts), 32):
            s, d = srcs[i:i + 32], dsts[i:i + 32]
            n = len(d)
            for a, b in zip(s, d):
                if b.dtype != torch.float32 or not b.is_contiguous() or (a is not None and (a.dtype != torch.float32 or not a.is_contiguous() or a.numel() != b.numel())):
                    raise RuntimeError("multi_copy: contiguous float32 tensors of matching sizes expected")
            self.call("ttk_multi_copy", n, (c_void_p * n)(*[ptr(a) for a in s]), (c_void_p * n)(*[ptr(b) for b in d]),
                      (c_int64 * n)(*[b.numel() for b in d]))

    @functools.lru_cache(maxsize=None)
    def anyc_partial_rows(self, pixels: int) -> int:
        return self.cdll.ttk_anyc_partial_rows(pixels)

    @functools.lru_cache(maxsize=None)
    def anyc_wgrad_scratch_bytes(self, kind: str, *shape) -> int:
        return getattr(self.cdll, f"ttk_anyc_{kind}_wgrad_scratch_bytes")(*shape)

    @functools.lru_cache(maxsize=None)
    def partial_rows_elementwise(self, items: int) -> int:
        return self.cdll.ttk_partial_rows_elementwise(items)

    @functools.lru_cache(maxsize=None)
    def partial_rows_dwconv(self, B, H, W, C, stride, backward) -> int:
        return self.cdll.ttk_partial_rows_dwconv(B, H, W, C, stride, int(backward))

    @functools.lru_cache(maxsize=None)
    def partial_rows_gemm(self, m: int, k: int | None = None, nout: int | None = None, dgrad: bool = False) -> int:
        if k is None:
            return self.cdll.ttk_partial_rows_gemm(m)
        return self.cdll.ttk_partial_rows_pwconv(m, k, nout, int(dgrad))


import threading

CAPTURE_LOCK = threading.RLock()

_lib: _Library | None = None


_raw_stream = torch._C._cuda_getCurrentRawStream
_cur_device = torch._C._cuda_getDevice


def lib() -> _Library:
    global _lib
    if _lib is None:
        _lib = _Library()
        if torch.cuda.is_available():
            _lib.clear_stale_error("library load")
    return _lib


def ptr(t: torch.Tensor | None):
    if t is None:
        return None
    if not t.is_cuda:
        raise RuntimeError("HIP entry point received a non-CUDA tensor")
    if not t.is_contiguous():
        raise RuntimeError("HIP entry point received a non-contiguous tensor")
    return t.data_ptr()


def check_tensors(ts, what="tensor"):
    for t in ts:
        if t is not None and not (t.is_cuda and t.is_contiguous()):
            raise RuntimeError(f"HIP entry point received a non-CUDA or non-contiguous {what}")


def fast_ptr(t: torch.Tensor | None):
    return None if t is None else t.data_ptr()


CHANNEL_BLOCK = 32


def to_blocks(t: torch.Tensor) -> torch.Tensor:
    C = t.shape[-1]
    if C <= CHANNEL_BLOCK:
        return t.contiguous()
    return t.reshape(-1, C // CHANNEL_BLOCK, CHANNEL_BLOCK).transpose(0, 1).contiguous().view(t.shape)


def to_blocks_any(t: torch.Tensor) -> torch.Tensor:
    C = t.shape[-1]
    if C % CHANNEL_BLOCK == 0:
        return to_blocks(t)
    full = C // CHANNEL_BLOCK * CHANNEL_BLOCK
    rows = t.reshape(-1, C)
    parts = [to_blocks(rows[:, :full]).reshape(-1)] if full else []
    return torch.cat(parts + [rows[:, full:].reshape(-1)]).view(t.shape)


def from_blocks_any(t: torch.Tensor) -> torch.Tensor:
    C = t.shape[-1]
    if C % CHANNEL_BLOCK == 0:
        return from_blocks(t)
    full = C // CHANNEL_BLOCK * CHANNEL_BLOCK
    flat = t.reshape(-1)
    M = flat.numel() // C
    tail = flat[M * full:].view(M, C - full)
    if not full:
        return tail.reshape(t.shape)
    return torch.cat([from_blocks(flat[:M * full].view(M, full)), tail], dim=1).reshape(t.shape)


def from_blocks(t: torch.Tensor) -> torch.Tensor:
    C = t.shape[-1]
    if C <= CHANNEL_BLOCK:
        return t
    return t.reshape(C // CHANNEL_BLOCK, -1, CHANNEL_BLOCK).transpose(0, 1).reshape(t.shape)


CHANNEL_BLOCK_BC = 64


def to_blocks64(t: torch.Tensor) -> torch.Tensor:
    C = t.shape[-1]
    if C <= CHANNEL_BLOCK_BC:
        return t.contiguous()
    return t.reshape(-1, C // CHANNEL_BLOCK_BC, CHANNEL_BLOCK_BC).transpose(0, 1).contiguous().view(t.shape)


def from_blocks64(t: torch.Tensor) -> torch.Tensor:
    C = t.shape[-1]
    if C <= CHANNEL_BLOCK_BC:
        return t
    return t.reshape(C // CHANNEL_BLOCK_BC, -1, CHANNEL_BLOCK_BC).transpose(0, 1).reshape(t.shape)


def exported_symbols() -> list[str]:
    return ["ttk_abi_version", "ttk_last_error_string", "ttk_clear_error", "ttk_partial_rows_elementwise",
            "ttk_partial_rows_gemm", "ttk_partial_rows_pwconv", "ttk_pwconv_tile_rows", "ttk_partial_rows_dwconv", "ttk_heads_num_rows", "ttk_pwconv_prepared_bytes",
            "ttk_pwconv_wgrad_partial_bytes", "ttk_pwconv_wgrad_scratch_bytes", "ttk_stem_wgrad_partial_bytes", "ttk_conv_wgrad_partial_bytes", "ttk_stem7_wgrad_partial_bytes",
            "ttk_pwconv1x1_bwd_fused_rows", "ttk_pwconv1x1_bwd_fused_partial_bytes", "ttk_bc_prepared_bytes", "ttk_bc_partial_rows_pw",
            "ttk_bc_partial_rows_dw", "ttk_bc_partial_rows_pool", "ttk_bc_pw_wgrad_scratch_bytes", "ttk_bc_pw_bwd_fused_rows",
            "ttk_bc_pw_bwd_fused_scratch_bytes", "ttk_bc_pw_wgrad_slices", "ttk_anyc_partial_rows", "ttk_anyc_stem_wgrad_scratch_bytes",
            "ttk_anyc_dw_wgrad_scratch_bytes", "ttk_anyc_pw_wgrad_scratch_bytes"] + list(_SIGNATURES)
```

neuralnet-tracker-traincode_amd/trackertraincode/backbones/mobilenet_v1.py:

```python
from __future__ import annotations

import math
import os
from typing import NamedTuple

import torch
import torch.nn as nn
import torch.nn.functional as F

import sys

from .. import _hip
from ..neuralnets.modelcomponents import BlurPool2D
from . import _mobilenet_bc

_THIS = sys.modules[__name__]

__all__ = ["MobileNet", "DepthWiseBlock"]

NormalizationLayer = nn.BatchNorm2d
ActivationFunc = nn.ReLU

_BLOCKS = (
    ("dw2_1", 32, 64, 1), ("dw2_2", 64, 128, 2), ("dw3_1", 128, 128, 1), ("dw3_2", 128, 256, 2),
    ("dw4_1", 256, 256, 1), ("dw4_2", 256, 512, 2), ("dw5_1", 512, 512, 1), ("dw5_2", 512, 512, 1),
    ("dw5_3", 512, 512, 1), ("dw5_4", 512, 512, 1), ("dw5_5", 512, 512, 1), ("dw5_6", 512, 1024, 2),
    ("dw6", 1024, 1024, 1),
)
_INTERMEDIATES = ("dw2_1", "dw3_1", "dw4_1", "dw5_5", "dw6")
_STEM_CHANNELS = 32


def _scaled_blocks(widen_factor):
    def ch(c):
        v = int(c * widen_factor)
        if v < 8 or v > 2048 or v % 8:
            raise ValueError(f"widen_factor={widen_factor} gives a channel count int({c} * {widen_factor}) = {v}; the HIP backbone takes "
                             "multiples of 8 in 8..2048 (e.g. widen_factor 0.25, 0.5, 0.75, 1.0, 1.5, 2.0)")
        return v
    return ch(_STEM_CHANNELS), tuple((name, ch(cin), ch(cout), stride) for name, cin, cout, stride in _BLOCKS)


def _tuned_c(c) -> bool:
    return 32 <= c <= 1024 and (c & (c - 1)) == 0


class DepthWiseBlock(nn.Module):

    def __init__(self, inplanes, planes, stride=1, momentum=0.1, stochastic_depth=None, use_blurpool=True):
        super().__init__()
        assert stride in (1, 2)
        self.inplanes, self.planes = inplanes, planes = int(inplanes), int(planes)
        self.stride = stride
        if stochastic_depth:
            raise NotImplementedError("stochastic_depth is never enabled by the reference's pose estimator")
        self.blurpool = stride == 2 and bool(use_blurpool)
        if self.blurpool:
            self.conv_dw = nn.Sequential(
                BlurPool2D(kernel_size=3, stride=2, channels=inplanes),
                nn.Conv2d(inplanes, inplanes, kernel_size=3, padding=1, stride=1, groups=inplanes, bias=False),
            )
        else:
            self.conv_dw = nn.Conv2d(inplanes, inplanes, kernel_size=3, padding=1, stride=stride, groups=inplanes, bias=False)
        self.bn_dw = NormalizationLayer(inplanes, momentum=momentum)
        self.conv_sep = nn.Conv2d(inplanes, planes, kernel_size=1, stride=1, padding=0, bias=False)
        self.bn_sep = NormalizationLayer(planes, momentum=momentum)
        self.relu = nn.ReLU(inplace=True)
        self.skip_connection = not (stride != 1 or inplanes != planes)
        self.stochastic_depth = None

    @property
    def dw_weight(self):
        return self.conv_dw[1].weight if self.blurpool else self.conv_dw.weight

    def forward(self, x):
        out = self.relu(self.bn_dw(self.conv_dw(x)))
        out = self.bn_sep(self.conv_sep(out))
        if self.skip_connection:
            out = out + x
        return self.relu(out)


_PRECISIONS = ("fp32", "bf16-compute")
_RETIRED = ("bf16", "bf16-all")
_DEFAULT_PRECISION = "fp32"


def _check_precision(mode):
    mode = {torch.float32: "fp32", "f32": "fp32"}.get(mode, mode)
    if mode in _RETIRED or mode is torch.bfloat16:
        raise ValueError(f'precision "{mode}" (bf16 storage under the fp32 kernels) was retired: it ran slower than fp32; use "bf16-compute"')
    if mode not in _PRECISIONS:
        raise ValueError(f'precision must be "fp32" or "bf16-compute", got {mode}')
    return mode


def set_activation_dtype(mode):
    global _DEFAULT_PRECISION
    _DEFAULT_PRECISION = _check_precision(mode)


def bf16_compute() -> bool:
    return _DEFAULT_PRECISION == "bf16-compute"


def get_activation_dtype():
    t = torch.bfloat16 if bf16_compute() else torch.float32
    return t, t


_BN_ROWS = 8


class _BnArena:

    def __init__(self, channels, device):
        self._buf = torch.zeros(sum(_BN_ROWS * c for c in channels), dtype=torch.float32, device=device)
        self._off = 0

    def take(self, C) -> torch.Tensor:
        n = _BN_ROWS * C
        blk = self._buf[self._off:self._off + n].view(_BN_ROWS, C)
        self._off += n
        return blk


class _Stage(NamedTuple):
    y: torch.Tensor
    bn: torch.Tensor
    skip: torch.Tensor | None


def _part_buffer(B, H, W, device, blur=False, blocks=_BLOCKS, c0=_STEM_CHANNELS):
    L = _hip.lib()
    need = 0
    h = (H + 1) // 2
    need = max(need, (L.partial_rows_elementwise(B * h * h * 8) if c0 == _STEM_CHANNELS else L.anyc_partial_rows(B * h * h)) * 2 * c0)
    for _, cin, cout, stride in blocks:
        ho = (h - 1) // stride + 1
        if _tuned_c(cin):
            need = max(need, L.partial_rows_dwconv(B, h, h, cin, stride, True) * 2 * cin)
            need = max(need, L.partial_rows_dwconv(B, h, h, cin, stride, False) * 2 * cin)
            if blur and stride == 2:
                need = max(need, L.partial_rows_dwconv(B, ho, ho, cin, 1, False) * 2 * cin, L.partial_rows_dwconv(B, ho, ho, cin, 1, True) * 2 * cin)
        else:
            need = max(need, L.anyc_partial_rows(B * h * h) * 2 * cin)
        if _tuned_c(cin) and _tuned_c(cout):
            need = max(need, L.partial_rows_gemm(B * ho * ho, cin, cout) * 2 * cout, L.partial_rows_gemm(B * ho * ho, cout, cin, True) * 2 * cin)
        else:
            need = max(need, L.partial_rows_gemm(B * ho * ho) * 2 * max(cin, cout))
        if _tuned_c(cout):
            need = max(need, L.partial_rows_elementwise(B * ho * ho * (cout // 4)) * 2 * cout)
        else:
            need = max(need, L.anyc_partial_rows(B * ho * ho) * 2 * cout)
        h = ho
    return torch.empty(need, dtype=torch.float32, device=device)


class _Ctx:
    __slots__ = ("x", "stages", "a_in", "part", "dims", "pool_skip", "wparams", "HW", "B", "prep", "bf", "gdt", "frozen", "blur", "blocks")


_IDENTITY_BN: dict = {}


def _identity_bn(C, device):
    key = (device.type, device.index, C)
    if key not in _IDENTITY_BN:
        t = torch.zeros((_BN_ROWS, C), dtype=torch.float32, device=device)
        t[0] = 1.0
        t[3] = 1.0
        _IDENTITY_BN[key] = t
    return _IDENTITY_BN[key].clone()


def _forward_impl(x, params, buffers, momentum, eps, training, frozen=False, blur=None, blocks=_BLOCKS):
    L = _hip.lib()
    blur = list(blur) if blur is not None else [None] * len(blocks)
    c0 = params[0].shape[0]
    _hip.check_tensors([x], "input")
    _hip.check_tensors(params, "parameter")
    _hip.check_tensors(buffers, "BatchNorm buffer")
    _hip.check_tensors(blur, "blur kernel")
    p = _hip.fast_ptr
    dev = x.device
    B, _, H, W = x.shape
    Ho, Wo = (H + 1) // 2, (W + 1) // 2
    part = _part_buffer(B, H, W, dev, any(b is not None for b in blur), blocks, c0)
    ctx = _Ctx()
    ctx.x, ctx.part, ctx.B, ctx.blocks = x, part, B, blocks
    ctx.blur = []
    ctx.frozen = frozen
    ctx.stages, ctx.a_in, ctx.dims = [], [], []
    act_dtype = torch.float32
    bf = 0
    ctx.bf, ctx.gdt = bf, torch.float32
    bns = _BnArena([c0] + [c for _, cin, cout, _ in blocks for c in (cin, cout)], dev)

    def pivot(bi):
        return p(buffers[3 * bi]) if _hip.bn_pivot() else None

    def finalize(bn, rows, C, count, gamma, beta, bi):
        rm, rv, nbt = buffers[3 * bi], buffers[3 * bi + 1], buffers[3 * bi + 2]
        if training:
            L.call("ttk_bn_fwd_finalize", p(part), pivot(bi), rows, C, count, p(gamma), p(beta), p(rm), p(rv), p(nbt),
                   float(momentum), float(eps), p(bn))
        else:
            L.call("ttk_bn_eval_prepare", p(gamma), p(beta), p(rm), p(rv), float(eps), C, p(bn))
            L.call("ttk_bn_frozen_bound", p(part), pivot(bi), rows, C, count, p(bn))

    part_arg = p(part)
    tuned_pw = [k for k, (_, cin, cout, _) in enumerate(blocks) if _tuned_c(cin) and _tuned_c(cout)]
    ctx.prep = [None] * len(blocks)
    if tuned_pw:
        sizes = [L.pwconv_prepared_bytes(blocks[k][1], blocks[k][2]) for k in tuned_pw]
        pool = torch.empty(sum(sizes), dtype=torch.uint8, device=dev)
        for k, t in zip(tuned_pw, torch.split(pool, sizes)):
            ctx.prep[k] = t
        L.pwconv_prepare_weights([params[3 + 6 * k + 3] for k in tuned_pw], [ctx.prep[k] for k in tuned_pw])
    y0 = torch.empty((B, Ho, Wo, c0), dtype=act_dtype, device=dev)
    bn = bns.take(c0)
    if c0 == _STEM_CHANNELS:
        L.call("ttk_stem_fwd", p(x), p(params[0]), p(y0), part_arg, pivot(0), B, H, W, bf)
        finalize(bn, L.partial_rows_elementwise(B * Ho * Wo * 8), 32, B * Ho * Wo, params[1], params[2], 0)
    else:
        L.call("ttk_anyc_stem_fwd", p(x), p(params[0]), p(y0), part_arg, pivot(0), B, H, W, c0)
        finalize(bn, L.anyc_partial_rows(B * Ho * Wo), c0, B * Ho * Wo, params[1], params[2], 0)
    prev = _Stage(y0, bn, None)
    ctx.stages.append(prev)
    h, w_ = Ho, Wo
    pi, bi = 3, 1
    def dw_fwd(yprev, bn_prev, skip_prev, a_out, w, y, pv, hh, ww, C, stride):
        if _tuned_c(C):
            L.call("ttk_dwconv3x3_fwd", p(yprev), p(bn_prev), p(skip_prev), p(a_out), p(w), p(y), part_arg, pv, B, hh, ww, C, stride, bf)
            return L.partial_rows_dwconv(B, hh, ww, C, stride, False)
        L.call("ttk_anyc_dw_fwd", p(yprev), p(bn_prev), p(skip_prev), p(a_out), p(w), p(y), part_arg, pv, B, hh, ww, C, stride)
        return L.anyc_partial_rows(B * ((hh - 1) // stride + 1) * ((ww - 1) // stride + 1))

    for name, cin, cout, stride in blocks:
        w_dw, g_dw, b_dw, w_pw, g_pw, b_pw = params[pi:pi + 6]
        pi += 6
        has_skip = stride == 1 and cin == cout
        ho, wo = (h - 1) // stride + 1, (w_ - 1) // stride + 1
        a_in = torch.empty_like(prev.y) if has_skip else None
        ydw = torch.empty((B, ho, wo, cin), dtype=act_dtype, device=dev)
        k = len(ctx.dims)
        if blur[k] is not None:
            t = torch.empty((B, ho, wo, cin), dtype=act_dtype, device=dev)
            dw_fwd(prev.y, prev.bn, prev.skip, None, blur[k], t, None, h, w_, cin, stride)
            st_t = _Stage(t, _identity_bn(cin, dev), None)
            dw_rows = dw_fwd(t, st_t.bn, None, None, w_dw, ydw, pivot(bi), ho, wo, cin, 1)
            ctx.blur.append((st_t, blur[k]))
        else:
            dw_rows = dw_fwd(prev.y, prev.bn, prev.skip, a_in, w_dw, ydw, pivot(bi), h, w_, cin, stride)
            ctx.blur.append(None)
        if _EXP_TENSOR_HOOK is not None:
            _EXP_TENSOR_HOOK("y", k, ydw)
        bn_dw = bns.take(cin)
        finalize(bn_dw, dw_rows, cin, B * ho * wo, g_dw, b_dw, bi)
        ypw = torch.empty((B, ho, wo, cout), dtype=act_dtype, device=dev)
        M = B * ho * wo
        if ctx.prep[k] is not None:
            L.call("ttk_pwconv1x1_fwd", p(ydw), p(bn_dw), None, p(ypw), part_arg, pivot(bi + 1), M, cin, cout, p(ctx.prep[k]), bf)
            pw_rows = L.partial_rows_gemm(M, cin, cout)
        else:
            L.call("ttk_anyc_pw_fwd", p(ydw), p(bn_dw), p(w_pw), p(ypw), part_arg, pivot(bi + 1), M, cin, cout)
            pw_rows = L.partial_rows_gemm(M)
        if _EXP_TENSOR_HOOK is not None:
            _EXP_TENSOR_HOOK("y", k, ypw)
        bn_pw = bns.take(cout)
        finalize(bn_pw, pw_rows, cout, M, g_pw, b_pw, bi + 1)
        bi += 2
        ctx.stages.append(_Stage(ydw, bn_dw, None))
        prev = _Stage(ypw, bn_pw, a_in)
        ctx.stages.append(prev)
        ctx.a_in.append(a_in)
        ctx.dims.append((h, w_, ho, wo, cin, cout, stride, has_skip))
        h, w_ = ho, wo
    C = prev.y.shape[-1]
    feat = torch.empty((B, C), dtype=torch.float32, device=dev)
    if _tuned_c(C):
        L.call("ttk_avgpool_fwd", p(prev.y), p(prev.bn), p(prev.skip), p(feat), B, h * w_, C, bf)
    else:
        L.call("ttk_anyc_avgpool_fwd", p(prev.y), p(prev.bn), p(prev.skip), p(feat), B, h * w_, C)
    ctx.HW = h * w_
    return feat, ctx


grad_ready_hook = None


_USE_WGRAD_STREAM = False
_DETERMINISTIC = os.environ.get("TTK_DETERMINISTIC", "0") != "0"
_FUSED_PW_BWD = True
_DW_WGRAD_ROWS = 2
_SIDE_STREAMS: dict = {}


def _side_stream(device):
    key = (device.type, device.index)
    if key not in _SIDE_STREAMS:
        _SIDE_STREAMS[key] = torch.cuda.Stream(device=device)
    return _SIDE_STREAMS[key]


_EXP_TENSOR_HOOK = None


def _backward_impl(ctx: _Ctx, gfeat, params):
    L = _hip.lib()
    _hip.check_tensors([gfeat], "gradient")
    _hip.check_tensors(params, "parameter")
    p = _hip.fast_ptr
    B, part, bf, blocks = ctx.B, ctx.part, ctx.bf, ctx.blocks
    offs, total = [], 0
    for q in params:
        offs.append(total)
        total += (q.numel() + 63) // 64 * 64
    offs.append(total)
    arena = torch.zeros(total, dtype=torch.float32, device=gfeat.device)
    grads = [arena[o:o + q.numel()].view(q.shape) for o, q in zip(offs, params)]

    def announce(first, last):
        grad_ready_hook(arena, [(params[i], offs[i], offs[i + 1]) for i in range(first, last)])
    last = ctx.stages[-1]
    C = last.y.shape[-1]

    def bwd_finalize(stage: _Stage, rows, count, gi):
        Cc = stage.y.shape[-1]
        if ctx.frozen:
            L.call("ttk_bn_bwd_frozen", p(stage.bn), Cc)
            return
        L.call("ttk_bn_bwd_finalize", p(part), rows, Cc, count, p(params[gi]), p(stage.bn), p(grads[gi]), p(grads[gi + 1]), 0)

    main = torch.cuda.current_stream(gfeat.device)
    side = _side_stream(gfeat.device) if (_USE_WGRAD_STREAM and not _DETERMINISTIC and all(q is not None for q in ctx.prep)) else None
    wg_scratch = None
    if _DETERMINISTIC:
        pw_dims = [d for d in ctx.dims if _tuned_c(d[4]) and _tuned_c(d[5])]
        dw_dims = [(d, bl) for d, bl in zip(ctx.dims, ctx.blur) if _tuned_c(d[4])]
        need = max([L.pwconv_wgrad_partial_bytes(B * d[2] * d[3], d[4], d[5]) for d in pw_dims] + [0])
        need = max(need, L.cdll.ttk_stem_wgrad_partial_bytes())
        need = max([need] + [L.cdll.ttk_pwconv1x1_bwd_fused_partial_bytes(B * d[2] * d[3], d[4], d[5]) for d in pw_dims])
        need = max([need] + [L.partial_rows_dwconv(B, d[0], d[1], d[4], d[6], True) * 9 * d[4] * 4 for d, _ in dw_dims])
        need = max([need] + [L.partial_rows_dwconv(B, d[2], d[3], d[4], 1, True) * 9 * d[4] * 4 for d, bl in dw_dims if bl is not None])
        wg_scratch = torch.empty(need // 4, dtype=torch.float32, device=gfeat.device)
    pw_need = max([L.pwconv_wgrad_scratch_bytes(B * d[2] * d[3], d[4], d[5]) for d in ctx.dims if _tuned_c(d[4]) and _tuned_c(d[5])] + [0])
    pw_scratch = wg_scratch if (wg_scratch is not None and wg_scratch.numel() * 4 >= pw_need) else (
        torch.empty(pw_need // 4, dtype=torch.float32, device=gfeat.device) if pw_need else None)
    keep = []
    dw_rows = wg_scratch
    rows_layers = [d for d, bl in zip(ctx.dims, ctx.blur) if bl is None and _tuned_c(d[4])]
    if dw_rows is None and _DW_WGRAD_ROWS and not ctx.frozen and rows_layers:
        need = max(L.partial_rows_dwconv(B, d[0], d[1], d[4], d[6], True) * 9 * d[4] for d in rows_layers)
        dw_rows = torch.empty(need, dtype=torch.float32, device=gfeat.device)

    _, _, H, W = ctx.x.shape
    c0 = ctx.stages[0].y.shape[-1]
    any_need = 0 if c0 == _STEM_CHANNELS else L.anyc_wgrad_scratch_bytes("stem", B, H, W, c0)
    for d, bl in zip(ctx.dims, ctx.blur):
        if not _tuned_c(d[4]):
            any_need = max(any_need, L.anyc_wgrad_scratch_bytes("dw", B, d[2], d[3], d[4]) if bl is not None else L.anyc_wgrad_scratch_bytes("dw", B, d[0], d[1], d[4]))
        if not (_tuned_c(d[4]) and _tuned_c(d[5])):
            any_need = max(any_need, L.anyc_wgrad_scratch_bytes("pw", B * d[2] * d[3], d[4], d[5]))
    any_scratch = torch.empty(any_need // 4, dtype=torch.float32, device=gfeat.device) if any_need else None

    g = torch.empty(last.y.shape, dtype=ctx.gdt, device=last.y.device)
    if _tuned_c(C):
        L.call("ttk_avgpool_bwd", p(gfeat), p(last.y), p(last.bn), p(last.skip), p(g), p(part), B, ctx.HW, C, bf)
        bwd_finalize(last, L.partial_rows_elementwise(B * ctx.HW * (C // 4)), B * ctx.HW, len(params) - 2)
    else:
        L.call("ttk_anyc_avgpool_bwd", p(gfeat), p(last.y), p(last.bn), p(last.skip), p(g), p(part), B, ctx.HW, C)
        bwd_finalize(last, L.anyc_partial_rows(B * ctx.HW), B * ctx.HW, len(params) - 2)
    if _EXP_TENSOR_HOOK is not None:
        _EXP_TENSOR_HOOK("g", len(blocks), g)

    for k in range(len(blocks) - 1, -1, -1):
        h, w_, ho, wo, cin, cout, stride, has_skip = ctx.dims[k]
        pi = 3 + 6 * k
        w_dw, w_pw = params[pi], params[pi + 3]
        st_prev, st_dw, st_pw = ctx.stages[2 * k], ctx.stages[2 * k + 1], ctx.stages[2 * k + 2]
        a_in = ctx.a_in[k]
        M = B * ho * wo
        dW = grads[pi + 3]
        g_dw = torch.empty(st_dw.y.shape, dtype=ctx.gdt, device=st_dw.y.device)
        pw_tuned = ctx.prep[k] is not None
        fused_rows = L.cdll.ttk_pwconv1x1_bwd_fused_rows(M, cin, cout) if (_FUSED_PW_BWD and bf == 0 and pw_tuned) else 0
        if not pw_tuned:
            L.call("ttk_anyc_pw_bwd_weight", p(g), p(st_pw.y), p(st_pw.bn), p(st_dw.y), p(st_dw.bn), p(dW), 0, p(any_scratch), M, cin, cout)
            L.call("ttk_anyc_pw_bwd_data", p(g), p(st_pw.y), p(st_pw.bn), p(w_pw), p(st_dw.y), p(st_dw.bn), p(g_dw), p(part), M, cin, cout)
            bwd_finalize(st_dw, L.partial_rows_gemm(M), M, pi + 1)
            if _EXP_TENSOR_HOOK is not None:
                _EXP_TENSOR_HOOK("g", k, g_dw)
        elif fused_rows:
            L.call("ttk_pwconv1x1_bwd_fused", p(g), p(st_pw.y), p(st_pw.bn), p(w_pw), p(ctx.prep[k]), p(st_dw.y), p(st_dw.bn), p(g_dw), p(dW),
                   p(wg_scratch), p(part), M, cin, cout)
            bwd_finalize(st_dw, fused_rows, M, pi + 1)
            if _EXP_TENSOR_HOOK is not None:
                _EXP_TENSOR_HOOK("g", k, g_dw)
        elif side is not None:
            ev = torch.cuda.Event()
            ev.record(main)
            side.wait_event(ev)
            with torch.cuda.stream(side):
                L.call("ttk_pwconv1x1_bwd_weight", p(g), p(st_pw.y), p(st_pw.bn), p(st_dw.y), p(st_dw.bn), p(dW),
                       p(pw_scratch) if L.pwconv_wgrad_scratch_bytes(M, cin, cout) else None, M, cin, cout, bf)
                if grad_ready_hook is not None:
                    done = torch.cuda.Event()
                    done.record(side)
            keep.append(g)
        else:
            L.call("ttk_pwconv1x1_bwd_weight", p(g), p(st_pw.y), p(st_pw.bn), p(st_dw.y), p(st_dw.bn), p(dW),
                   p(wg_scratch) if wg_scratch is not None else (p(pw_scratch) if L.pwconv_wgrad_scratch_bytes(M, cin, cout) else None), M, cin, cout, bf)
        if pw_tuned and not fused_rows:
            L.call("ttk_pwconv1x1_bwd_data", p(g), p(st_pw.y), p(st_pw.bn), None, p(st_dw.y), p(st_dw.bn), p(g_dw), p(part), M,
                   cin, cout, p(ctx.prep[k]), bf)
            bwd_finalize(st_dw, L.partial_rows_gemm(M, cout, cin, True), M, pi + 1)
            if _EXP_TENSOR_HOOK is not None:
                _EXP_TENSOR_HOOK("g", k, g_dw)
        dWd = grads[pi]
        g_prev = torch.empty(st_prev.y.shape, dtype=ctx.gdt, device=st_prev.y.device)
        gi_prev = pi - 2 if k > 0 else 1
        if not _tuned_c(cin):
            if ctx.blur[k] is not None:
                st_t, w_blur = ctx.blur[k]
                g_t = torch.empty(st_t.y.shape, dtype=ctx.gdt, device=st_t.y.device)
                L.call("ttk_anyc_dw_bwd_data", p(g_dw), p(st_dw.y), p(st_dw.bn), p(w_dw), None, p(st_t.y), p(st_t.bn), None, None, p(g_t),
                       p(part), p(dWd), 0, p(any_scratch), B, ho, wo, cin, 1)
                L.call("ttk_bn_bwd_frozen", p(st_t.bn), cin)
                L.call("ttk_anyc_dw_bwd_data", p(g_t), p(st_t.y), p(st_t.bn), p(w_blur), None, p(st_prev.y), p(st_prev.bn), p(st_prev.skip),
                       None, p(g_prev), p(part), None, 0, None, B, h, w_, cin, stride)
            else:
                L.call("ttk_anyc_dw_bwd_data", p(g_dw), p(st_dw.y), p(st_dw.bn), p(w_dw), p(g) if has_skip else None, p(st_prev.y),
                       p(st_prev.bn), p(st_prev.skip), p(a_in), p(g_prev), p(part), p(dWd), 0, p(any_scratch), B, h, w_, cin, stride)
            bwd_finalize(st_prev, L.anyc_partial_rows(B * h * w_), B * h * w_, gi_prev)
        elif ctx.blur[k] is not None:
            st_t, w_blur = ctx.blur[k]
            g_t = torch.empty(st_t.y.shape, dtype=ctx.gdt, device=st_t.y.device)
            L.call("ttk_dwconv3x3_bwd_data", p(g_dw), p(st_dw.y), p(st_dw.bn), p(w_dw), None, p(st_t.y), p(st_t.bn), None, None, p(g_t),
                   p(part), p(dWd), 1, p(wg_scratch), B, ho, wo, cin, 1, bf)
            L.call("ttk_bn_bwd_frozen", p(st_t.bn), cin)
            L.call("ttk_dwconv3x3_bwd_data", p(g_t), p(st_t.y), p(st_t.bn), p(w_blur), None, p(st_prev.y), p(st_prev.bn), p(st_prev.skip),
                   None, p(g_prev), p(part), None, 0, None, B, h, w_, cin, stride, bf)
            bwd_finalize(st_prev, L.partial_rows_dwconv(B, h, w_, cin, stride, True), B * h * w_, pi - 2 if k > 0 else 1)
        elif _DW_WGRAD_ROWS == 2 and not _DETERMINISTIC and not ctx.frozen:
            rows, gi = L.partial_rows_dwconv(B, h, w_, cin, stride, True), (pi - 2 if k > 0 else 1)
            L.call("ttk_dwconv3x3_bwd_data", p(g_dw), p(st_dw.y), p(st_dw.bn), p(w_dw), p(g) if has_skip else None, p(st_prev.y),
                   p(st_prev.bn), p(st_prev.skip), p(a_in), p(g_prev), p(part), p(dWd), 2, p(dw_rows), B, h, w_, cin, stride, bf)
            L.call("ttk_bc_bn_bwd_finalize_fold", p(part), rows, cin, B * h * w_, p(params[gi]), p(st_prev.bn), p(grads[gi]), p(grads[gi + 1]), 0,
                   p(dw_rows), rows, 9 * cin, p(dWd), 1)
        else:
            L.call("ttk_dwconv3x3_bwd_data", p(g_dw), p(st_dw.y), p(st_dw.bn), p(w_dw), p(g) if has_skip else None, p(st_prev.y),
                   p(st_prev.bn), p(st_prev.skip), p(a_in), p(g_prev), p(part), p(dWd), 1,
                   p(dw_rows if (_DW_WGRAD_ROWS == 1 and not ctx.frozen) else wg_scratch), B, h, w_, cin, stride, bf)
            bwd_finalize(st_prev, L.partial_rows_dwconv(B, h, w_, cin, stride, True), B * h * w_, pi - 2 if k > 0 else 1)
        g = g_prev
        if _EXP_TENSOR_HOOK is not None:
            _EXP_TENSOR_HOOK("g", k, g)
        if grad_ready_hook is not None:
            if side is not None:
                main.wait_event(done)
            announce(pi, pi + 6)
    st0 = ctx.stages[0]
    if c0 == _STEM_CHANNELS:
        L.call("ttk_stem_bwd_weight", p(g), p(st0.y), p(st0.bn), p(ctx.x), p(grads[0]), 1, p(wg_scratch), B, H, W, bf)
    else:
        L.call("ttk_anyc_stem_bwd_weight", p(g), p(st0.y), p(st0.bn), p(ctx.x), p(grads[0]), 0, p(any_scratch), B, H, W, c0)
    if grad_ready_hook is not None:
        announce(0, 3)
    if side is not None:
        main.wait_stream(side)
        keep.clear()
    return grads


class _MobileNetFn(torch.autograd.Function):

    @staticmethod
    def forward(ctx, x, momentum, eps, buffers, frozen, blur, precision, blocks, *params):
        if precision == "bf16-compute":
            feat, c = _mobilenet_bc.forward_impl(_THIS, x, params, buffers, momentum, eps, training=not frozen, frozen=frozen, blur=blur)
        else:
            feat, c = _forward_impl(x, params, buffers, momentum, eps, training=not frozen, frozen=frozen, blur=blur, blocks=blocks)
        ctx.c = c
        ctx.nparams = len(params)
        ctx.save_for_backward(*params)
        return feat

    @staticmethod
    def backward(ctx, gfeat):
        params = ctx.saved_tensors
        if ctx.c.bf == "bc":
            grads = _mobilenet_bc.backward_impl(_THIS, ctx.c, gfeat.contiguous(), params)
        else:
            grads = _backward_impl(ctx.c, gfeat.contiguous(), params)
        ctx.c = None
        return (None, None, None, None, None, None, None, None, *grads)


class MobileNet(nn.Module):

    def __init__(self, num_classes=1000, widen_factor=1.0, input_channel=1, momentum=0.1, dropout=0.0,
                 use_blurpool=False, return_only_featuremap=False):
        super().__init__()
        if input_channel != 1:
            raise NotImplementedError("the HIP backbone is built for input_channel=1 (the pose estimator's configuration, models.py:220)")
        self.widen_factor = widen_factor
        c0, self._blocks = _scaled_blocks(widen_factor)
        if return_only_featuremap:
            raise NotImplementedError("return_only_featuremap is not used by the pose estimator")

        def block(inplanes, planes, stride=1):
            return DepthWiseBlock(inplanes, planes, stride=stride, momentum=momentum, use_blurpool=use_blurpool)

        self.use_blurpool = bool(use_blurpool)
        self.precision = None
        self.conv1 = nn.Conv2d(input_channel, c0, kernel_size=5, stride=2, padding=2, bias=False)
        self.bn1 = NormalizationLayer(c0, momentum=momentum)
        self.relu = ActivationFunc(inplace=True)
        for name, cin, cout, stride in self._blocks:
            setattr(self, name, block(cin, cout, stride))
        self.avgpool = nn.AdaptiveAvgPool2d(1)
        self.num_features = int(1024 * widen_factor)
        self.num_intermediate_features = [cout for name, _, cout, _ in self._blocks if name in _INTERMEDIATES]
        if num_classes:
            self.drop = nn.Dropout(p=dropout) if dropout > 0.0 else nn.Identity()
            self.fc = nn.Linear(self.num_features, num_classes)
        for m in self.modules():
            if isinstance(m, nn.Conv2d):
                n = m.kernel_size[0] * m.kernel_size[1] * m.out_channels
                m.weight.data.normal_(0, math.sqrt(2.0 / n))

    def set_precision(self, mode):
        mode = None if mode is None else _check_precision(mode)
        self._check_width_precision(mode)
        self.precision = mode
        return self

    def effective_precision(self) -> str:
        return self.precision if getattr(self, "precision", None) is not None else _DEFAULT_PRECISION

    def _check_width_precision(self, mode):
        if mode == "bf16-compute" and self._blocks != _BLOCKS:
            raise ValueError(f'precision "bf16-compute" is built for widen_factor=1.0 only (its kernels work on 64-channel blocks); this backbone '
                             f'has widen_factor={self.widen_factor}: use "fp32"')

    def kernel_plan(self):
        fam = lambda ok: "tuned" if ok else "anyc"
        plan = [("conv1", fam(self.conv1.out_channels == _STEM_CHANNELS))]
        for name, cin, cout, _ in self._blocks:
            plan.append((f"{name}.conv_dw", fam(_tuned_c(cin))))
            plan.append((f"{name}.conv_sep", fam(_tuned_c(cin) and _tuned_c(cout))))
        plan.append(("avgpool", fam(_tuned_c(self.num_features))))
        return plan

    def _bns(self):
        yield self.bn1
        for name, *_ in self._blocks:
            blk = getattr(self, name)
            yield blk.bn_dw
            yield blk.bn_sep

    def _flat_params(self):
        ps = [self.conv1.weight, self.bn1.weight, self.bn1.bias]
        for name, *_ in self._blocks:
            b = getattr(self, name)
            ps += [b.dw_weight, b.bn_dw.weight, b.bn_dw.bias, b.conv_sep.weight, b.bn_sep.weight, b.bn_sep.bias]
        return ps

    def _blur_weights(self):
        if not self.use_blurpool:
            return None
        return [getattr(self, name).conv_dw[0].depthwise_weight() if getattr(self, name).blurpool else None for name, *_ in self._blocks]

    def _flat_buffers(self):
        out = []
        for bn in self._bns():
            out += [bn.running_mean, bn.running_var, bn.num_batches_tracked]
        return out

    def _check(self, x):
        if x.dtype != torch.float32 or x.dim() != 4 or x.shape[1] != 1:
            raise ValueError(f"expected float32 [B,1,H,W] input, got {tuple(x.shape)} {x.dtype}")
        moms = {bn.momentum for bn in self._bns()}
        epss = {bn.eps for bn in self._bns()}
        if len(moms) != 1 or len(epss) != 1 or None in moms:
            raise NotImplementedError("all BatchNorm layers must share one momentum/eps")
        return moms.pop(), epss.pop()

    def forward_features(self, x: torch.Tensor) -> torch.Tensor:
        if not x.is_cuda:
            return self._forward_torch(x)[0]
        momentum, eps = self._check(x)
        self._check_width_precision(self.effective_precision())
        x = x.contiguous()
        bn_training = [bn.training for bn in self._bns()]
        if self.training and all(bn_training):
            return _MobileNetFn.apply(x, momentum, eps, self._flat_buffers(), False, self._blur_weights(), self.effective_precision(), self._blocks, *self._flat_params())
        if any(bn_training):
            raise NotImplementedError("mixed train/eval BatchNorm layers are not supported by the fused backbone")
        if torch.is_grad_enabled() and any(p.requires_grad for p in self._flat_params()):
            if any(p.requires_grad for bn in self._bns() for p in bn.parameters()):
                raise NotImplementedError("eval-mode BatchNorm layers with trainable weight / bias are not built: freeze them "
                                          "(modelcomponents.freeze_norm_stats) or put the layers in training mode")
            return _MobileNetFn.apply(x, momentum, eps, self._flat_buffers(), True, self._blur_weights(), self.effective_precision(), self._blocks, *self._flat_params())
        if self.effective_precision() == "bf16-compute":
            feat, _ = _mobilenet_bc.forward_impl(_THIS, x, [q.detach() for q in self._flat_params()], self._flat_buffers(), momentum, eps, False,
                                                 blur=self._blur_weights())
        else:
            feat, _ = _forward_impl(x, [q.detach() for q in self._flat_params()], self._flat_buffers(), momentum, eps, False, blur=self._blur_weights(),
                                    blocks=self._blocks)
        return feat

    def forward(self, x):
        if not x.is_cuda:
            return self._forward_torch(x)
        feat = self.forward_features(x)
        if hasattr(self, "fc"):
            feat = self.fc(self.drop(feat))
        return feat, self._intermediates(x)

    @torch.no_grad()
    def _intermediates(self, x):
        momentum, eps = self._check(x)
        bufs = [b.clone() for b in self._flat_buffers()]
        training = self.training
        _, c = _forward_impl(x.contiguous(), [q.detach() for q in self._flat_params()], bufs, momentum, eps, training, blur=self._blur_weights(),
                             blocks=self._blocks)
        L, p = _hip.lib(), _hip.ptr
        outs = []
        for k, (name, *_r) in enumerate(self._blocks):
            if name in _INTERMEDIATES:
                st = c.stages[2 * k + 2]
                a = torch.empty_like(st.y)
                L.call("ttk_bn_act" if _tuned_c(a.shape[-1]) else "ttk_anyc_bn_act", p(st.y), p(st.bn), p(st.skip), p(a), a.numel() // a.shape[-1], a.shape[-1])
                outs.append(a.permute(0, 3, 1, 2))
        return outs

    def _forward_torch(self, x):
        if self.training:
            raise RuntimeError("the MI355X training path needs CUDA tensors; CPU tensors are accepted in eval() mode only")
        x = self.relu(self.bn1(self.conv1(x)))
        outs = []
        for name, *_ in self._blocks:
            x = getattr(self, name)(x)
            if name in _INTERMEDIATES:
                outs.append(x)
        x = self.avgpool(x)
        x = x.view(x.size(0), -1)
        if hasattr(self, "fc"):
            x = self.fc(self.drop(x))
        return x, outs

    def prepare_finetune(self):
        return [[*ch.parameters()] for ch in self.children()]
```

Baseline: 71810 crops/s.

## Recompute residual skip from raw pre-BN input instead of storing a_in

For the first residual block of stages dw3_1 and dw4_1, the materialized post-activation input buffer a_in is no longer written. The dwconv forward/backward and avgpool kernels gain a raw-skip variant that applies the previous stage's BN+activation to the raw tensor on the fly. This saves a full activation write in forward and the matching reads, at the cost of extra BN arithmetic and smaller unroll factors, which may change register pressure.

```diff
diff --git a/include/ttk.h b/include/ttk.h
--- a/include/ttk.h
+++ b/include/ttk.h
@@ -10,7 +10,7 @@
 
 typedef void* ttk_stream_t;
 
-#define TTK_ABI_VERSION 31
+#define TTK_ABI_VERSION 32
 
 enum {
   TTK_BN_SCALE = 0,
@@ -68,6 +68,14 @@
                            const float* skip_prev, const float* a_in, float* g_prev, float* part,
                            float* dw, int dw_accumulate, float* dw_partial, int B, int H, int W, int C,
                            int stride, int act_bf16, ttk_stream_t stream);
+int ttk_dwconv3x3_fwd_rawskip(const float* yprev, const float* bn_prev, const float* skip_raw, const float* skip_bn, float* a_out,
+                              const float* w, float* y, float* part, const float* pivot, int B, int H, int W, int C,
+                              int stride, ttk_stream_t stream);
+int ttk_dwconv3x3_bwd_data_rawskip(const float* g_dw, const float* y_dw, const float* bn_dw, const float* w,
+                                   const float* skip_grad, const float* yprev, float* bn_prev,
+                                   const float* skip_raw, const float* skip_bn, float* g_prev, float* part,
+                                   float* dw, int dw_accumulate, float* dw_partial, int B, int H, int W, int C,
+                                   int stride, ttk_stream_t stream);
 
 int ttk_pwconv1x1_fwd(const float* ydw, const float* bn_dw, const float* w, float* y, float* part, const float* pivot,
                       int64_t M, int Cin, int Cout, void* wsplit, int act_bf16, ttk_stream_t stream);
@@ -93,6 +101,10 @@
                     int C, int act_bf16, ttk_stream_t stream);
 int ttk_avgpool_bwd(const float* gfeat, const float* y, float* bn, const float* skip, float* g,
                     float* part, int B, int HW, int C, int act_bf16, ttk_stream_t stream);
+int ttk_avgpool_fwd_rawskip(const float* y, const float* bn, const float* skip_raw, const float* skip_bn, float* feat, int B, int HW,
+                            int C, ttk_stream_t stream);
+int ttk_avgpool_bwd_rawskip(const float* gfeat, const float* y, float* bn, const float* skip_raw, const float* skip_bn, float* g,
+                            float* part, int B, int HW, int C, ttk_stream_t stream);
 int ttk_bn_act(const float* y, const float* bn, const float* skip, float* a, int64_t rows, int C,
                ttk_stream_t stream);
 
diff --git a/neuralnet-tracker-traincode_amd/csrc/dwconv_tiled.hip b/neuralnet-tracker-traincode_amd/csrc/dwconv_tiled.hip
--- a/neuralnet-tracker-traincode_amd/csrc/dwconv_tiled.hip
+++ b/neuralnet-tracker-traincode_amd/csrc/dwconv_tiled.hip
@@ -168,13 +168,17 @@
   }
 }
 
-template <int S, bool SKIP, int SL, bool CARRY>
+enum { kSkipNone = 0, kSkipStored = 1, kSkipRaw = 2 };
+__device__ __forceinline__ const float* only_ptr(const float* p) { return p; }
+
+template <int S, int SKIP, int SL, bool CARRY, typename... BnSkip>
 __global__ void __launch_bounds__(kBlock) __attribute__((amdgpu_waves_per_eu(TTK_DW_WGS_PER_CU, TTK_DW_WGS_PER_CU)))
 dw_fwd_tiled_k(const float* __restrict__ yprev, const float* __restrict__ bn_prev,
                                                           const float* __restrict__ skip_prev, float* __restrict__ a_out,
                                                           const float* __restrict__ w, float* __restrict__ y,
                                                           float* __restrict__ part, const float* __restrict__ pivot, int B, int H, int W, int C,
-                                                          int Ho, int Wo, int R, int nbands, int nslabs, int NI_, int NCT_, int TW) {
+                                                          int Ho, int Wo, int R, int nbands, int nslabs, int NI_, int NCT_, int TW, BnSkip... bn_skip) {
+  static_assert(sizeof...(BnSkip) == (SKIP == kSkipRaw ? 1 : 0), "bn_skip: the raw residual form's one extra argument");
   extern __shared__ __attribute__((aligned(16))) float lds[];
   constexpr int kSlab = SL, kSlabQuads = SL / 4, kPixSlots = kBlock / kSlabQuads, kQs = ilog2(kSlabQuads), kPs = ilog2(SL);
   const int tid = threadIdx.x, q = tid & (kSlabQuads - 1), slot = tid >> kQs;
@@ -184,6 +188,8 @@
   SlabWeights wr;
   wr.load(w, c0);
   const BnApply4 bn = BnApply4::load(bn_prev, C, c0);
+  BnApply4 bns = bn;
+  if constexpr (SKIP == kSkipRaw) bns = BnApply4::load(only_ptr(bn_skip...), C, c0);
   const float4 pv = pivot ? ld4(pivot + c0) : f4(0.f);
   D4 s1{0.0, 0.0, 0.0, 0.0}, s2{0.0, 0.0, 0.0, 0.0};
   const int NI = CARRY ? 1 : NI_, NCT = CARRY ? 1 : NCT_;
@@ -229,7 +235,7 @@
     }
     const int nstage = nimg * ((int)PI - ov * Wp) * kSlabQuads;
     const unsigned ovpix = (unsigned)(ov * Wp);
-    constexpr int kFwdU = SKIP ? kFwdUSkip : (S == 2 ? kFwdUPlain2 : (CARRY ? kFwdUPlain - 1 : kFwdUPlain));
+    constexpr int kFwdU = SKIP ? (SKIP == kSkipRaw && S == 1 && CARRY ? kFwdUSkip - 1 : kFwdUSkip) : (S == 2 ? kFwdUPlain2 : (CARRY ? kFwdUPlain - 1 : kFwdUPlain));
     for (int e = tid; e < nstage; e += kFwdU * kBlock) {
       float4 yv[kFwdU], sk[SKIP ? kFwdU : 1];
       unsigned off[kFwdU];
@@ -255,7 +261,8 @@
         if (ee >= nstage) break;
         float4 a = f4(0.f);
         if (in[u]) {
-          if constexpr (SKIP) a = bn.act(yv[u], sk[u]);
+          if constexpr (SKIP == kSkipRaw) a = bn.act(yv[u], bns.act(sk[u]));
+          else if constexpr (SKIP == kSkipStored) a = bn.act(yv[u], sk[u]);
           else a = bn.act(yv[u]);
           if (S == 1 && a_out && rows[u]) st4(aotile + off[u], a);
         }
@@ -294,7 +301,7 @@
 #ifndef TTK_DW_BWD_LEAN_PIX2
 #define TTK_DW_BWD_LEAN_PIX2 4
 #endif
-template <int S, int SL, bool LEAN, bool CARRY>
+template <int S, int SL, bool LEAN, bool CARRY, typename... BnSkip>
 __global__ void __launch_bounds__(kBlock) __attribute__((amdgpu_waves_per_eu(TTK_DW_WGS_PER_CU, TTK_DW_WGS_PER_CU)))
 dw_bwd_tiled_k(const float* __restrict__ g_dw, const float* __restrict__ y_dw,
                                                           const float* __restrict__ bn_dw, const float* __restrict__ w,
@@ -303,7 +310,9 @@
                                                           const float* __restrict__ skip_prev, const float* __restrict__ a_in,
                                                           float* __restrict__ g_prev, float* __restrict__ part,
                                                           float* __restrict__ dwgrad, float* __restrict__ dw_partial, int B, int H, int W, int C, int Ho, int Wo,
-                                                          int R, int nbands, int nslabs, int stage_floats, int NI_, int NCT_, int TW, int ring) {
+                                                          int R, int nbands, int nslabs, int stage_floats, int NI_, int NCT_, int TW, int ring, BnSkip... bn_skip) {
+  constexpr bool RAWSKIP = sizeof...(BnSkip) == 1;
+  static_assert(sizeof...(BnSkip) <= 1 && !(RAWSKIP && LEAN), "bn_skip: the raw residual form's one extra argument");
   extern __shared__ __attribute__((aligned(16))) float lds[];
   const int NI = CARRY ? 1 : NI_, NCT = CARRY ? 1 : NCT_;
   constexpr int kSlab = SL, kSlabQuads = SL / 4, kPixSlots = kBlock / kSlabQuads, kQs = ilog2(kSlabQuads), kPs = ilog2(SL);
@@ -318,6 +327,8 @@
   static_assert(SL == kCB, "a slab is one channel block of the activation layout");
   constexpr int cshift = 5;
   const BnApply4 bnp = BnApply4::load(bn_prev, C, c0);
+  BnApply4 bns = bnp;
+  if constexpr (RAWSKIP) bns = BnApply4::load(only_ptr(bn_skip...), C, c0);
   const BnGrad4 bg = BnGrad4::load(bn_dw, C, c0);
   D4 s1{0.0, 0.0, 0.0, 0.0}, s2{0.0, 0.0, 0.0, 0.0};
   float gmx = 0.f;
@@ -355,7 +366,7 @@
     __syncthreads();
     const unsigned ovpix = (unsigned)(ov * Wp);
     const int nstage = nimg * ((int)PI - (int)ovpix) * kSlabQuads;
-    constexpr int kBwdU = TTK_DW_BWD_U;
+    constexpr int kBwdU = (RAWSKIP && S == 1 && !CARRY) ? TTK_DW_BWD_U - 2 : TTK_DW_BWD_U;
     for (int e = tid; e < nstage; e += kBwdU * kBlock) {
       float4 gv[kBwdU], yv[kBwdU];
       bool in[kBwdU];
@@ -427,7 +438,8 @@
         const float* dyimg = lds + (__umul24(imgs[j], PI) << kPs);
         const float4 yp = yps[j], raw = raws[j], sg = sgs[j];
         float4 a;
-        if (!LEAN && a_in) a = raw;
+        if constexpr (RAWSKIP) a = bnp.act(yp, bns.act(raw));
+        else if (!LEAN && a_in) a = raw;
         else a = (!LEAN && skip_prev) ? bnp.act(yp, raw) : bnp.act(yp);
         float4 G = f4(0.f);
 #pragma unroll
@@ -510,57 +522,96 @@
   return dw_tiling(B, H, W, C, stride, backward != 0).rows;
 }
 
-int ttk_dwconv3x3_fwd(const float* yprev, const float* bn_prev, const float* skip_prev, float* a_out, const float* w, float* y,
-                      float* part, const float* pivot, int B, int H, int W, int C, int stride, int act_bf16, ttk_stream_t stream) {
-  TTK_REQUIRE(yprev && bn_prev && w && y, "dwconv3x3_fwd: null pointer");
-  TTK_REQUIRE(dw_shape_ok2(B, H, W, C, stride), "dwconv3x3_fwd: unsupported shape B=%d H=%d W=%d C=%d stride=%d (C: power of two in 32..1024, W <= 256)", B, H, W, C, stride);
-  TTK_REQUIRE(!(a_out && stride != 1), "dwconv3x3_fwd: a_out requires stride 1");
-  TTK_REQUIRE_FP32_STORAGE(act_bf16, "dwconv3x3_fwd");
+static int dw_fwd_launch(const char* name, bool raw, const float* yprev, const float* bn_prev, const float* skip_prev, const float* skip_bn, float* a_out,
+                         const float* w, float* y, float* part, const float* pivot, int B, int H, int W, int C, int stride, int act_bf16, ttk_stream_t stream) {
+  TTK_REQUIRE(yprev && bn_prev && w && y && (!raw || (skip_prev && skip_bn)), "%s: null pointer", name);
+  TTK_REQUIRE(dw_shape_ok2(B, H, W, C, stride), "%s: unsupported shape B=%d H=%d W=%d C=%d stride=%d (C: power of two in 32..1024, W <= 256)", name, B, H, W, C, stride);
+  TTK_REQUIRE(!(a_out && stride != 1), "%s: a_out requires stride 1", name);
+  TTK_REQUIRE((act_bf16 & 3) == 0, "%s: bf16 activation storage under the fp32 kernels was retired (round 6): use the bf16-compute path (ttk_bc_*)", name);
   const int Ho = (H - 1) / stride + 1, Wo = (W - 1) / stride + 1;
   const DwTiling t = dw_tiling(B, H, W, C, stride, false);
-  TTK_REQUIRE((int64_t)((B + t.NI - 1) / t.NI) * t.nbands * t.NCT < ((int64_t)1 << 31), "dwconv3x3_fwd: too many tiles for 32-bit indexing");
+  TTK_REQUIRE((int64_t)((B + t.NI - 1) / t.NI) * t.nbands * t.NCT < ((int64_t)1 << 31), "%s: too many tiles for 32-bit indexing", name);
   const size_t stage = (size_t)t.NI * t.stage_rows * ((t.NCT > 1 ? t.TW : W) + 2) * t.SL;
   const size_t sm = (stage + 16 * t.SL) * sizeof(float);
   with_flag(stride == 2, [&](auto s2) {
-    with_flag(skip_prev != nullptr, [&](auto skip) {
-      with_flag(t.carry != 0, [&](auto carry) {
-        hipLaunchKernelGGL((dw_fwd_tiled_k<decltype(s2)::value ? 2 : 1, decltype(skip)::value, kCB, decltype(carry)::value>), dim3(t.grid), dim3(kBlock), sm,
-                           (hipStream_t)stream, yprev, bn_prev, skip_prev, a_out, w, y, part, pivot, B, H, W, C, Ho, Wo, t.R, t.nbands, t.nslabs, t.NI,
-                           t.NCT, t.TW);
-      });
+    with_flag(t.carry != 0, [&](auto carry) {
+      constexpr int S = decltype(s2)::value ? 2 : 1;
+      constexpr bool CARRY = decltype(carry)::value;
+      if (raw) {
+        hipLaunchKernelGGL((dw_fwd_tiled_k<S, kSkipRaw, kCB, CARRY, const float*>), dim3(t.grid), dim3(kBlock), sm, (hipStream_t)stream, yprev, bn_prev, skip_prev,
+                           a_out, w, y, part, pivot, B, H, W, C, Ho, Wo, t.R, t.nbands, t.nslabs, t.NI, t.NCT, t.TW, skip_bn);
+      } else {
+        with_flag(skip_prev != nullptr, [&](auto skip) {
+          hipLaunchKernelGGL((dw_fwd_tiled_k<S, decltype(skip)::value ? kSkipStored : kSkipNone, kCB, CARRY>), dim3(t.grid), dim3(kBlock), sm, (hipStream_t)stream, yprev, bn_prev, skip_prev,
+                             a_out, w, y, part, pivot, B, H, W, C, Ho, Wo, t.R, t.nbands, t.nslabs, t.NI, t.NCT, t.TW);
+        });
+      }
     });
   });
-  TTK_LAUNCH_CHECK("dwconv3x3_fwd");
+  TTK_LAUNCH_CHECK(name);
+}
+
+int ttk_dwconv3x3_fwd(const float* yprev, const float* bn_prev, const float* skip_prev, float* a_out, const float* w, float* y,
+                      float* part, const float* pivot, int B, int H, int W, int C, int stride, int act_bf16, ttk_stream_t stream) {
+  return dw_fwd_launch("dwconv3x3_fwd", false, yprev, bn_prev, skip_prev, nullptr, a_out, w, y, part, pivot, B, H, W, C, stride, act_bf16, stream);
+}
+
+int ttk_dwconv3x3_fwd_rawskip(const float* yprev, const float* bn_prev, const float* skip_raw, const float* skip_bn, float* a_out, const float* w, float* y,
+                              float* part, const float* pivot, int B, int H, int W, int C, int stride, ttk_stream_t stream) {
+  return dw_fwd_launch("dwconv3x3_fwd_rawskip", true, yprev, bn_prev, skip_raw, skip_bn, a_out, w, y, part, pivot, B, H, W, C, stride, 0, stream);
+}
+
+static int dw_bwd_launch(const char* name, bool raw, const float* g_dw, const float* y_dw, const float* bn_dw, const float* w, const float* skip_grad,
+                         const float* yprev, float* bn_prev, const float* skip_prev, const float* skip_bn, const float* a_in, float* g_prev, float* part, float* dw,
+                         int dw_accumulate, float* dw_partial, int B, int H, int W, int C, int stride, int act_bf16, ttk_stream_t stream) {
+  TTK_REQUIRE(g_dw && y_dw && bn_dw && w && yprev && bn_prev && g_prev && (!raw || (skip_prev && skip_bn)), "%s: null pointer", name);
+  TTK_REQUIRE(dw_shape_ok2(B, H, W, C, stride), "%s: unsupported shape", name);
+  TTK_REQUIRE(!(skip_grad && stride != 1), "%s: residual gradient requires stride 1", name);
+  TTK_REQUIRE((act_bf16 & 3) == 0, "%s: bf16 activation storage under the fp32 kernels was retired (round 6): use the bf16-compute path (ttk_bc_*)", name);
+  const int Ho = (H - 1) / stride + 1, Wo = (W - 1) / stride + 1;
+  const DwTiling t = dw_tiling(B, H, W, C, stride, true);
+  TTK_REQUIRE((int64_t)((B + t.NI - 1) / t.NI) * t.nbands * t.NCT < ((int64_t)1 << 31), "%s: too many tiles for 32-bit indexing", name);
+  const size_t stage = (size_t)t.NI * t.stage_rows * ((t.NCT > 1 ? t.TW : Wo) + 2) * t.SL;
+  const size_t sm = (stage + 4 * 9 * t.SL + 9 * t.SL) * sizeof(float);
+  hipStream_t st = (hipStream_t)stream;
+  if (!dw) dw_partial = nullptr;
+  TTK_REQUIRE(dw_accumulate != 2 || dw_partial, "%s: dw_accumulate = 2 (rows folded by the caller) needs dw and dw_partial", name);
+  if (dw && !dw_accumulate && !dw_partial) hipLaunchKernelGGL(zero_fill_k, dim3((9 * C + 255) / 256), dim3(256), 0, st, dw, (int64_t)9 * C);
+  with_flag(stride == 2, [&](auto s2) {
+    with_flag(t.carry != 0, [&](auto carry) {
+      constexpr int S = decltype(s2)::value ? 2 : 1;
+      constexpr bool CARRY = decltype(carry)::value;
+      if (raw) {
+        hipLaunchKernelGGL((dw_bwd_tiled_k<S, kCB, false, CARRY, const float*>), dim3(t.grid), dim3(kBlock), sm, st, g_dw, y_dw, bn_dw, w, skip_grad, yprev, bn_prev,
+                           skip_prev, a_in, g_prev, part, dw, dw_partial, B, H, W, C, Ho, Wo, t.R, t.nbands, t.nslabs, (int)stage, t.NI, t.NCT, t.TW, t.stage_rows,
+                           skip_bn);
+      } else {
+        with_flag(!a_in && !skip_prev && !skip_grad, [&](auto lean) {
+          hipLaunchKernelGGL((dw_bwd_tiled_k<S, kCB, decltype(lean)::value, CARRY>), dim3(t.grid), dim3(kBlock), sm, st, g_dw, y_dw, bn_dw, w, skip_grad, yprev,
+                             bn_prev, skip_prev, a_in, g_prev, part, dw, dw_partial, B, H, W, C, Ho, Wo, t.R, t.nbands, t.nslabs, (int)stage, t.NI, t.NCT, t.TW,
+                             t.stage_rows);
+        });
+      }
+    });
+  });
+  if (dw_partial && dw_accumulate != 2) launch_fold_partials(dw_partial, t.rows, (int64_t)9 * C, dw, dw_accumulate, st);
+  TTK_LAUNCH_CHECK(name);
 }
 
 int ttk_dwconv3x3_bwd_data(const float* g_dw, const float* y_dw, const float* bn_dw, const float* w, const float* skip_grad,
                            const float* yprev, float* bn_prev, const float* skip_prev, const float* a_in, float* g_prev,
                            float* part, float* dw, int dw_accumulate, float* dw_partial, int B, int H, int W, int C, int stride,
                            int act_bf16, ttk_stream_t stream) {
-  TTK_REQUIRE(g_dw && y_dw && bn_dw && w && yprev && bn_prev && g_prev, "dwconv3x3_bwd_data: null pointer");
-  TTK_REQUIRE(dw_shape_ok2(B, H, W, C, stride), "dwconv3x3_bwd_data: unsupported shape");
-  TTK_REQUIRE(!(skip_grad && stride != 1), "dwconv3x3_bwd_data: residual gradient requires stride 1");
-  TTK_REQUIRE_FP32_STORAGE(act_bf16, "dwconv3x3_bwd_data");
-  const int Ho = (H - 1) / stride + 1, Wo = (W - 1) / stride + 1;
-  const DwTiling t = dw_tiling(B, H, W, C, stride, true);
-  TTK_REQUIRE((int64_t)((B + t.NI - 1) / t.NI) * t.nbands * t.NCT < ((int64_t)1 << 31), "dwconv3x3_bwd_data: too many tiles for 32-bit indexing");
-  const size_t stage = (size_t)t.NI * t.stage_rows * ((t.NCT > 1 ? t.TW : Wo) + 2) * t.SL;
-  const size_t sm = (stage + 4 * 9 * t.SL + 9 * t.SL) * sizeof(float);
-  hipStream_t st = (hipStream_t)stream;
-  if (!dw) dw_partial = nullptr;
-  TTK_REQUIRE(dw_accumulate != 2 || dw_partial, "dwconv3x3_bwd_data: dw_accumulate = 2 (rows folded by the caller) needs dw and dw_partial");
-  if (dw && !dw_accumulate && !dw_partial) hipLaunchKernelGGL(zero_fill_k, dim3((9 * C + 255) / 256), dim3(256), 0, st, dw, (int64_t)9 * C);
-  with_flag(stride == 2, [&](auto s2) {
-    with_flag(!a_in && !skip_prev && !skip_grad, [&](auto lean) {
-      with_flag(t.carry != 0, [&](auto carry) {
-        hipLaunchKernelGGL((dw_bwd_tiled_k<decltype(s2)::value ? 2 : 1, kCB, decltype(lean)::value, decltype(carry)::value>), dim3(t.grid), dim3(kBlock), sm, st,
-                           g_dw, y_dw, bn_dw, w, skip_grad, yprev, bn_prev, skip_prev, a_in, g_prev, part, dw, dw_partial, B, H, W, C, Ho, Wo, t.R,
-                           t.nbands, t.nslabs, (int)stage, t.NI, t.NCT, t.TW, t.stage_rows);
-      });
-    });
-  });
-  if (dw_partial && dw_accumulate != 2) launch_fold_partials(dw_partial, t.rows, (int64_t)9 * C, dw, dw_accumulate, st);
-  TTK_LAUNCH_CHECK("dwconv3x3_bwd_data");
-}
-
-}
+  return dw_bwd_launch("dwconv3x3_bwd_data", false, g_dw, y_dw, bn_dw, w, skip_grad, yprev, bn_prev, skip_prev, nullptr, a_in, g_prev, part, dw, dw_accumulate,
+                       dw_partial, B, H, W, C, stride, act_bf16, stream);
+}
+
+int ttk_dwconv3x3_bwd_data_rawskip(const float* g_dw, const float* y_dw, const float* bn_dw, const float* w, const float* skip_grad,
+                                   const float* yprev, float* bn_prev, const float* skip_raw, const float* skip_bn, float* g_prev,
+                                   float* part, float* dw, int dw_accumulate, float* dw_partial, int B, int H, int W, int C, int stride,
+                                   ttk_stream_t stream) {
+  return dw_bwd_launch("dwconv3x3_bwd_data_rawskip", true, g_dw, y_dw, bn_dw, w, skip_grad, yprev, bn_prev, skip_raw, skip_bn, nullptr, g_prev, part, dw,
+                       dw_accumulate, dw_partial, B, H, W, C, stride, 0, stream);
+}
+
+}
diff --git a/neuralnet-tracker-traincode_amd/csrc/pool.hip b/neuralnet-tracker-traincode_amd/csrc/pool.hip
--- a/neuralnet-tracker-traincode_amd/csrc/pool.hip
+++ b/neuralnet-tracker-traincode_amd/csrc/pool.hip
@@ -8,9 +8,13 @@
   return act_off(m, c, M);
 }
 
+__device__ __forceinline__ const float* only_ptr(const float* p) { return p; }
+
+template <typename... BnSkip>
 __global__ void __launch_bounds__(kBlock) avgpool_fwd_k(const float* __restrict__ y, const float* __restrict__ bnp,
                                                          const float* __restrict__ skip,
-                                                         float* __restrict__ feat, int B, int HW, int C, int rows_layout) {
+                                                         float* __restrict__ feat, int B, int HW, int C, int rows_layout, BnSkip... bn_skip) {
+  constexpr bool RAW = sizeof...(BnSkip) == 1;
   const int quads = C >> 2;
   const int64_t items = (int64_t)B * quads;
   const float inv = 1.0f / (float)HW;
@@ -18,23 +22,30 @@
     const int c4 = (int)(idx % quads);
     const int n = (int)(idx / quads);
     const BnApply4 bn = BnApply4::load(bnp, C, 4 * c4);
+    BnApply4 bs = bn;
+    if constexpr (RAW) bs = BnApply4::load(only_ptr(bn_skip...), C, 4 * c4);
     float4 s = f4(0.f);
     for (int p = 0; p < HW; ++p) {
       const int64_t m = (int64_t)n * HW + p;
       const size_t off = pool_off(rows_layout, m, 4 * c4, (int64_t)B * HW, C);
-      s = add4(s, skip ? bn.act(ld4(y + off), ld4(skip + off)) : bn.act(ld4(y + off)));
+      if constexpr (RAW) s = add4(s, bn.act(ld4(y + off), bs.act(ld4(skip + off))));
+      else s = add4(s, skip ? bn.act(ld4(y + off), ld4(skip + off)) : bn.act(ld4(y + off)));
     }
     st4(feat + (size_t)n * C + 4 * c4, make_float4(s.x * inv, s.y * inv, s.z * inv, s.w * inv));
   }
 }
 
+template <typename... BnSkip>
 __global__ void __launch_bounds__(kBlock) avgpool_bwd_k(const float* __restrict__ gfeat, const float* __restrict__ y,
                                                          float* __restrict__ bnp, const float* __restrict__ skip, float* __restrict__ g,
-                                                         float* __restrict__ part, int B, int HW, int C, int qshift, int rows_layout) {
+                                                         float* __restrict__ part, int B, int HW, int C, int qshift, int rows_layout, BnSkip... bn_skip) {
+  constexpr bool RAW = sizeof...(BnSkip) == 1;
   extern __shared__ __attribute__((aligned(16))) float smem[];
   const int quads = C >> 2;
   const int c4 = threadIdx.x & (quads - 1);
   const BnApply4 bn = BnApply4::load(bnp, C, 4 * c4);
+  BnApply4 bs = bn;
+  if constexpr (RAW) bs = BnApply4::load(only_ptr(bn_skip...), C, 4 * c4);
   const float inv = 1.0f / (float)HW;
   const int64_t items = ((int64_t)B * HW) << qshift;
   float4 s1 = f4(0.f), s2 = f4(0.f);
@@ -43,7 +54,9 @@
     const int n = (int)((unsigned)(idx >> qshift) / (unsigned)HW);
     const size_t off = pool_off(rows_layout, idx >> qshift, 4 * c4, (int64_t)B * HW, C);
     const float4 yv = ld4(y + off);
-    const float4 a = skip ? bn.act(yv, ld4(skip + off)) : bn.act(yv);
+    float4 a;
+    if constexpr (RAW) a = bn.act(yv, bs.act(ld4(skip + off)));
+    else a = skip ? bn.act(yv, ld4(skip + off)) : bn.act(yv);
     float4 gv = ld4(gfeat + (size_t)n * C + 4 * c4);
     gv = mask4(make_float4(gv.x * inv, gv.y * inv, gv.z * inv, gv.w * inv), a);
     st4(g + off, gv);
@@ -74,28 +87,58 @@
 
 extern "C" {
 
+static int avgpool_fwd_launch(const char* name, const float* y, const float* bn, const float* skip, const float* skip_bn, float* feat, int B, int HW, int C,
+                              int act_bf16, ttk_stream_t stream) {
+  TTK_REQUIRE(y && bn && feat, "%s: null pointer", name);
+  TTK_REQUIRE(B > 0 && HW > 0 && C >= 32 && C <= 1024 && (C & (C - 1)) == 0, "%s: unsupported shape B=%d HW=%d C=%d", name, B, HW, C);
+  TTK_REQUIRE((act_bf16 & 3) == 0, "%s: bf16 activation storage under the fp32 kernels was retired (round 6): use the bf16-compute path (ttk_bc_*)", name);
+  const int64_t items = (int64_t)B * (C / 4);
+  if (skip_bn)
+    hipLaunchKernelGGL((avgpool_fwd_k<const float*>), dim3(elementwise_grid(items)), dim3(kBlock), 0, (hipStream_t)stream, y, bn, skip, feat, B, HW, C,
+                       pool_layout(act_bf16), skip_bn);
+  else
+    hipLaunchKernelGGL((avgpool_fwd_k<>), dim3(elementwise_grid(items)), dim3(kBlock), 0, (hipStream_t)stream, y, bn, skip, feat, B, HW, C,
+                       pool_layout(act_bf16));
+  TTK_LAUNCH_CHECK(name);
+}
+
 int ttk_avgpool_fwd(const float* y, const float* bn, const float* skip, float* feat, int B, int HW,
                     int C, int act_bf16, ttk_stream_t stream) {
-  TTK_REQUIRE(y && bn && feat, "avgpool_fwd: null pointer");
-  TTK_REQUIRE(B > 0 && HW > 0 && C >= 32 && C <= 1024 && (C & (C - 1)) == 0, "avgpool_fwd: unsupported shape B=%d HW=%d C=%d", B, HW, C);
-  TTK_REQUIRE_FP32_STORAGE(act_bf16, "avgpool_fwd");
-  const int64_t items = (int64_t)B * (C / 4);
-  hipLaunchKernelGGL(avgpool_fwd_k, dim3(elementwise_grid(items)), dim3(kBlock), 0, (hipStream_t)stream, y, bn, skip, feat, B, HW, C,
-                     pool_layout(act_bf16));
-  TTK_LAUNCH_CHECK("avgpool_fwd");
+  return avgpool_fwd_launch("avgpool_fwd", y, bn, skip, nullptr, feat, B, HW, C, act_bf16, stream);
+}
+
+int ttk_avgpool_fwd_rawskip(const float* y, const float* bn, const float* skip_raw, const float* skip_bn, float* feat, int B, int HW,
+                            int C, ttk_stream_t stream) {
+  TTK_REQUIRE(skip_raw && skip_bn, "avgpool_fwd_rawskip: null pointer");
+  return avgpool_fwd_launch("avgpool_fwd_rawskip", y, bn, skip_raw, skip_bn, feat, B, HW, C, 0, stream);
+}
+
+static int avgpool_bwd_launch(const char* name, const float* gfeat, const float* y, float* bn, const float* skip, const float* skip_bn, float* g, float* part,
+                              int B, int HW, int C, int act_bf16, ttk_stream_t stream) {
+  TTK_REQUIRE(gfeat && y && bn && g, "%s: null pointer", name);
+  TTK_REQUIRE(B > 0 && HW > 0 && C >= 32 && C <= 1024 && (C & (C - 1)) == 0, "%s: unsupported shape", name);
+  TTK_REQUIRE((int64_t)B * HW < (int64_t)1 << 31, "%s: too many pixels for 32-bit indexing", name);
+  TTK_REQUIRE((act_bf16 & 3) == 0, "%s: bf16 activation storage under the fp32 kernels was retired (round 6): use the bf16-compute path (ttk_bc_*)", name);
+  const int qs = log2i_(C / 4);
+  const int64_t items = ((int64_t)B * HW) << qs;
+  if (skip_bn)
+    hipLaunchKernelGGL((avgpool_bwd_k<const float*>), dim3(elementwise_grid(items)), dim3(kBlock), 2 * (size_t)C * sizeof(float), (hipStream_t)stream, gfeat, y,
+                       bn, skip, g, part, B, HW, C, qs, pool_layout(act_bf16), skip_bn);
+  else
+    hipLaunchKernelGGL((avgpool_bwd_k<>), dim3(elementwise_grid(items)), dim3(kBlock), 2 * (size_t)C * sizeof(float), (hipStream_t)stream, gfeat, y, bn,
+                       skip, g, part, B, HW, C, qs, pool_layout(act_bf16));
+  TTK_LAUNCH_CHECK(name);
 }
 
 int ttk_avgpool_bwd(const float* gfeat, const float* y, float* bn, const float* skip, float* g,
                     float* part, int B, int HW, int C, int act_bf16, ttk_stream_t stream) {
-  TTK_REQUIRE(gfeat && y && bn && g, "avgpool_bwd: null pointer");
-  TTK_REQUIRE(B > 0 && HW > 0 && C >= 32 && C <= 1024 && (C & (C - 1)) == 0, "avgpool_bwd: unsupported shape");
-  TTK_REQUIRE((int64_t)B * HW < (int64_t)1 << 31, "avgpool_bwd: too many pixels for 32-bit indexing");
-  TTK_REQUIRE_FP32_STORAGE(act_bf16, "avgpool_bwd");
-  const int qs = log2i_(C / 4);
-  const int64_t items = ((int64_t)B * HW) << qs;
-  hipLaunchKernelGGL(avgpool_bwd_k, dim3(elementwise_grid(items)), dim3(kBlock), 2 * (size_t)C * sizeof(float), (hipStream_t)stream, gfeat, y, bn,
-                     skip, g, part, B, HW, C, qs, pool_layout(act_bf16));
-  TTK_LAUNCH_CHECK("avgpool_bwd");
+  return avgpool_bwd_launch("avgpool_bwd", gfeat, y, bn, skip, nullptr, g, part, B, HW, C, act_bf16, stream);
+}
+
+int ttk_avgpool_bwd_rawskip(const float* gfeat, const float* y, float* bn, const float* skip_raw, const float* skip_bn, float* g,
+                            float* part, int B, int HW, int C, ttk_stream_t stream) {
+  TTK_REQUIRE(skip_raw && skip_bn, "avgpool_bwd_rawskip: null pointer");
+  return avgpool_bwd_launch("avgpool_bwd_rawskip", gfeat, y, bn, skip_raw, skip_bn, g, part, B, HW, C, 0, stream);
 }
 
 }
diff --git a/neuralnet-tracker-traincode_amd/trackertraincode/_hip.py b/neuralnet-tracker-traincode_amd/trackertraincode/_hip.py
--- a/neuralnet-tracker-traincode_amd/trackertraincode/_hip.py
+++ b/neuralnet-tracker-traincode_amd/trackertraincode/_hip.py
@@ -23,6 +23,8 @@
     "ttk_stem_bwd_weight": [_P, _P, _P, _P, _P, _I, _P, _I, _I, _I, _I],
     "ttk_dwconv3x3_fwd": [_P] * 8 + [_I] * 6,
     "ttk_dwconv3x3_bwd_data": [_P] * 12 + [_I, _P] + [_I] * 6,
+    "ttk_dwconv3x3_fwd_rawskip": [_P] * 9 + [_I] * 5,
+    "ttk_dwconv3x3_bwd_data_rawskip": [_P] * 12 + [_I, _P] + [_I] * 5,
     "ttk_pwconv1x1_fwd": [_P, _P, _P, _P, _P, _P, _L, _I, _I, _P, _I],
     "ttk_pwconv1x1_bwd_data": [_P] * 8 + [_L, _I, _I, _P, _I],
     "ttk_pwconv1x1_bwd_weight": [_P] * 7 + [_L, _I, _I, _I],
@@ -31,6 +33,8 @@
     "ttk_transpose": [_P, _P, _I, _I],
     "ttk_avgpool_fwd": [_P, _P, _P, _P, _I, _I, _I, _I],
     "ttk_avgpool_bwd": [_P, _P, _P, _P, _P, _P, _I, _I, _I, _I],
+    "ttk_avgpool_fwd_rawskip": [_P, _P, _P, _P, _P, _I, _I, _I],
+    "ttk_avgpool_bwd_rawskip": [_P, _P, _P, _P, _P, _P, _P, _I, _I, _I],
     "ttk_bn_act": [_P, _P, _P, _P, _L, _I],
     "ttk_stem7_fwd": [_P, _P, _P, _P, _P, _I, _I, _I],
     "ttk_stem7_bwd_weight": [_P, _P, _P, _P, _P, _P, _I, _I, _I],
@@ -116,7 +120,7 @@
     "ttk_anyc_bn_act": [_P, _P, _P, _P, _L, _I],
 }
 
-ABI_VERSION = 31
+ABI_VERSION = 32
 
 
 BN_PIVOT = True
diff --git a/neuralnet-tracker-traincode_amd/trackertraincode/backbones/mobilenet_v1.py b/neuralnet-tracker-traincode_amd/trackertraincode/backbones/mobilenet_v1.py
--- a/neuralnet-tracker-traincode_amd/trackertraincode/backbones/mobilenet_v1.py
+++ b/neuralnet-tracker-traincode_amd/trackertraincode/backbones/mobilenet_v1.py
@@ -129,6 +129,7 @@
     y: torch.Tensor
     bn: torch.Tensor
     skip: torch.Tensor | None
+    skip_bn: torch.Tensor | None = None
 
 
 def _part_buffer(B, H, W, device, blur=False, blocks=_BLOCKS, c0=_STEM_CHANNELS):
@@ -230,9 +231,13 @@
     ctx.stages.append(prev)
     h, w_ = Ho, Wo
     pi, bi = 3, 1
-    def dw_fwd(yprev, bn_prev, skip_prev, a_out, w, y, pv, hh, ww, C, stride):
+    def dw_fwd(st, a_out, w, y, pv, hh, ww, C, stride):
+        yprev, bn_prev, skip_prev = st.y, st.bn, st.skip
         if _tuned_c(C):
-            L.call("ttk_dwconv3x3_fwd", p(yprev), p(bn_prev), p(skip_prev), p(a_out), p(w), p(y), part_arg, pv, B, hh, ww, C, stride, bf)
+            if st.skip_bn is not None:
+                L.call("ttk_dwconv3x3_fwd_rawskip", p(yprev), p(bn_prev), p(skip_prev), p(st.skip_bn), p(a_out), p(w), p(y), part_arg, pv, B, hh, ww, C, stride)
+            else:
+                L.call("ttk_dwconv3x3_fwd", p(yprev), p(bn_prev), p(skip_prev), p(a_out), p(w), p(y), part_arg, pv, B, hh, ww, C, stride, bf)
             return L.partial_rows_dwconv(B, hh, ww, C, stride, False)
         L.call("ttk_anyc_dw_fwd", p(yprev), p(bn_prev), p(skip_prev), p(a_out), p(w), p(y), part_arg, pv, B, hh, ww, C, stride)
         return L.anyc_partial_rows(B * ((hh - 1) // stride + 1) * ((ww - 1) // stride + 1))
@@ -242,17 +247,18 @@
         pi += 6
         has_skip = stride == 1 and cin == cout
         ho, wo = (h - 1) // stride + 1, (w_ - 1) // stride + 1
-        a_in = torch.empty_like(prev.y) if has_skip else None
+        head = has_skip and prev.skip is None and _tuned_c(cin) and (_ELIDE_HEAD_INPUT is True or (bool(_ELIDE_HEAD_INPUT) and name in _ELIDE_HEAD_INPUT))
+        a_in = torch.empty_like(prev.y) if (has_skip and not head) else None
         ydw = torch.empty((B, ho, wo, cin), dtype=act_dtype, device=dev)
         k = len(ctx.dims)
         if blur[k] is not None:
             t = torch.empty((B, ho, wo, cin), dtype=act_dtype, device=dev)
-            dw_fwd(prev.y, prev.bn, prev.skip, None, blur[k], t, None, h, w_, cin, stride)
+            dw_fwd(prev, None, blur[k], t, None, h, w_, cin, stride)
             st_t = _Stage(t, _identity_bn(cin, dev), None)
-            dw_rows = dw_fwd(t, st_t.bn, None, None, w_dw, ydw, pivot(bi), ho, wo, cin, 1)
+            dw_rows = dw_fwd(st_t, None, w_dw, ydw, pivot(bi), ho, wo, cin, 1)
             ctx.blur.append((st_t, blur[k]))
         else:
-            dw_rows = dw_fwd(prev.y, prev.bn, prev.skip, a_in, w_dw, ydw, pivot(bi), h, w_, cin, stride)
+            dw_rows = dw_fwd(prev, a_in, w_dw, ydw, pivot(bi), h, w_, cin, stride)
             ctx.blur.append(None)
         if _EXP_TENSOR_HOOK is not None:
             _EXP_TENSOR_HOOK("y", k, ydw)
@@ -272,14 +278,16 @@
         finalize(bn_pw, pw_rows, cout, M, g_pw, b_pw, bi + 1)
         bi += 2
         ctx.stages.append(_Stage(ydw, bn_dw, None))
-        prev = _Stage(ypw, bn_pw, a_in)
+        prev = _Stage(ypw, bn_pw, skip=prev.y, skip_bn=prev.bn) if head else _Stage(ypw, bn_pw, a_in)
         ctx.stages.append(prev)
         ctx.a_in.append(a_in)
         ctx.dims.append((h, w_, ho, wo, cin, cout, stride, has_skip))
         h, w_ = ho, wo
     C = prev.y.shape[-1]
     feat = torch.empty((B, C), dtype=torch.float32, device=dev)
-    if _tuned_c(C):
+    if _tuned_c(C) and prev.skip_bn is not None:
+        L.call("ttk_avgpool_fwd_rawskip", p(prev.y), p(prev.bn), p(prev.skip), p(prev.skip_bn), p(feat), B, h * w_, C)
+    elif _tuned_c(C):
         L.call("ttk_avgpool_fwd", p(prev.y), p(prev.bn), p(prev.skip), p(feat), B, h * w_, C, bf)
     else:
         L.call("ttk_anyc_avgpool_fwd", p(prev.y), p(prev.bn), p(prev.skip), p(feat), B, h * w_, C)
@@ -293,6 +301,7 @@
 _USE_WGRAD_STREAM = False
 _DETERMINISTIC = os.environ.get("TTK_DETERMINISTIC", "0") != "0"
 _FUSED_PW_BWD = True
+_ELIDE_HEAD_INPUT = ("dw3_1", "dw4_1")
 _DW_WGRAD_ROWS = 2
 _SIDE_STREAMS: dict = {}
 
@@ -367,13 +376,24 @@
 
     g = torch.empty(last.y.shape, dtype=ctx.gdt, device=last.y.device)
     if _tuned_c(C):
-        L.call("ttk_avgpool_bwd", p(gfeat), p(last.y), p(last.bn), p(last.skip), p(g), p(part), B, ctx.HW, C, bf)
+        if last.skip_bn is not None:
+            L.call("ttk_avgpool_bwd_rawskip", p(gfeat), p(last.y), p(last.bn), p(last.skip), p(last.skip_bn), p(g), p(part), B, ctx.HW, C)
+        else:
+            L.call("ttk_avgpool_bwd", p(gfeat), p(last.y), p(last.bn), p(last.skip), p(g), p(part), B, ctx.HW, C, bf)
         bwd_finalize(last, L.partial_rows_elementwise(B * ctx.HW * (C // 4)), B * ctx.HW, len(params) - 2)
     else:
         L.call("ttk_anyc_avgpool_bwd", p(gfeat), p(last.y), p(last.bn), p(last.skip), p(g), p(part), B, ctx.HW, C)
         bwd_finalize(last, L.anyc_partial_rows(B * ctx.HW), B * ctx.HW, len(params) - 2)
     if _EXP_TENSOR_HOOK is not None:
         _EXP_TENSOR_HOOK("g", len(blocks), g)
+
+    def dw_bwd(g_dw, st_dw, w, skip_grad, st_prev, a_in, g_prev, dw, acc, rows, hh, ww, C, stride):
+        if st_prev.skip_bn is not None and a_in is None:
+            L.call("ttk_dwconv3x3_bwd_data_rawskip", p(g_dw), p(st_dw.y), p(st_dw.bn), p(w), p(skip_grad), p(st_prev.y), p(st_prev.bn), p(st_prev.skip),
+                   p(st_prev.skip_bn), p(g_prev), p(part), p(dw), acc, p(rows), B, hh, ww, C, stride)
+        else:
+            L.call("ttk_dwconv3x3_bwd_data", p(g_dw), p(st_dw.y), p(st_dw.bn), p(w), p(skip_grad), p(st_prev.y), p(st_prev.bn),
+                   p(st_prev.skip if st_prev.skip_bn is None else None), p(a_in), p(g_prev), p(part), p(dw), acc, p(rows), B, hh, ww, C, stride, bf)
 
     for k in range(len(blocks) - 1, -1, -1):
         h, w_, ho, wo, cin, cout, stride, has_skip = ctx.dims[k]
@@ -437,22 +457,18 @@
         elif ctx.blur[k] is not None:
             st_t, w_blur = ctx.blur[k]
             g_t = torch.empty(st_t.y.shape, dtype=ctx.gdt, device=st_t.y.device)
-            L.call("ttk_dwconv3x3_bwd_data", p(g_dw), p(st_dw.y), p(st_dw.bn), p(w_dw), None, p(st_t.y), p(st_t.bn), None, None, p(g_t),
-                   p(part), p(dWd), 1, p(wg_scratch), B, ho, wo, cin, 1, bf)
+            dw_bwd(g_dw, st_dw, w_dw, None, st_t, None, g_t, dWd, 1, wg_scratch, ho, wo, cin, 1)
             L.call("ttk_bn_bwd_frozen", p(st_t.bn), cin)
-            L.call("ttk_dwconv3x3_bwd_data", p(g_t), p(st_t.y), p(st_t.bn), p(w_blur), None, p(st_prev.y), p(st_prev.bn), p(st_prev.skip),
-                   None, p(g_prev), p(part), None, 0, None, B, h, w_, cin, stride, bf)
+            dw_bwd(g_t, st_t, w_blur, None, st_prev, None, g_prev, None, 0, None, h, w_, cin, stride)
             bwd_finalize(st_prev, L.partial_rows_dwconv(B, h, w_, cin, stride, True), B * h * w_, pi - 2 if k > 0 else 1)
         elif _DW_WGRAD_ROWS == 2 and not _DETERMINISTIC and not ctx.frozen:
             rows, gi = L.partial_rows_dwconv(B, h, w_, cin, stride, True), (pi - 2 if k > 0 else 1)
-            L.call("ttk_dwconv3x3_bwd_data", p(g_dw), p(st_dw.y), p(st_dw.bn), p(w_dw), p(g) if has_skip else None, p(st_prev.y),
-                   p(st_prev.bn), p(st_prev.skip), p(a_in), p(g_prev), p(part), p(dWd), 2, p(dw_rows), B, h, w_, cin, stride, bf)
+            dw_bwd(g_dw, st_dw, w_dw, g if has_skip else None, st_prev, a_in, g_prev, dWd, 2, dw_rows, h, w_, cin, stride)
             L.call("ttk_bc_bn_bwd_finalize_fold", p(part), rows, cin, B * h * w_, p(params[gi]), p(st_prev.bn), p(grads[gi]), p(grads[gi + 1]), 0,
                    p(dw_rows), rows, 9 * cin, p(dWd), 1)
         else:
-            L.call("ttk_dwconv3x3_bwd_data", p(g_dw), p(st_dw.y), p(st_dw.bn), p(w_dw), p(g) if has_skip else None, p(st_prev.y),
-                   p(st_prev.bn), p(st_prev.skip), p(a_in), p(g_prev), p(part), p(dWd), 1,
-                   p(dw_rows if (_DW_WGRAD_ROWS == 1 and not ctx.frozen) else wg_scratch), B, h, w_, cin, stride, bf)
+            dw_bwd(g_dw, st_dw, w_dw, g if has_skip else None, st_prev, a_in, g_prev, dWd, 1,
+                   dw_rows if (_DW_WGRAD_ROWS == 1 and not ctx.frozen) else wg_scratch, h, w_, cin, stride)
             bwd_finalize(st_prev, L.partial_rows_dwconv(B, h, w_, cin, stride, True), B * h * w_, pi - 2 if k > 0 else 1)
         g = g_prev
         if _EXP_TENSOR_HOOK is not None:
@@ -632,8 +648,13 @@
         for k, (name, *_r) in enumerate(self._blocks):
             if name in _INTERMEDIATES:
                 st = c.stages[2 * k + 2]
+                skip = st.skip
+                if st.skip_bn is not None:
+                    skip = torch.empty_like(st.skip)
+                    L.call("ttk_bn_act", p(st.skip), p(st.skip_bn), None, p(skip), skip.numel() // skip.shape[-1], skip.shape[-1])
+                    skip = _hip.to_blocks(skip)
                 a = torch.empty_like(st.y)
-                L.call("ttk_bn_act" if _tuned_c(a.shape[-1]) else "ttk_anyc_bn_act", p(st.y), p(st.bn), p(st.skip), p(a), a.numel() // a.shape[-1], a.shape[-1])
+                L.call("ttk_bn_act" if _tuned_c(a.shape[-1]) else "ttk_anyc_bn_act", p(st.y), p(st.bn), p(skip), p(a), a.numel() // a.shape[-1], a.shape[-1])
                 outs.append(a.permute(0, 3, 1, 2))
         return outs
 
```

Result: faster. 73270 crops/s (median of 6 runs) (+2.0%).
